# om-ai-lab/OmChat

Hardware: AMD Instinct MI355X
Metric: images/sec prefill + decode tokens/sec, OmChat-13B TP=1/8; p50 TTFT (higher is better)
Workload: dtype bf16

## Files before the change

### include/omchat_hip.h

```cpp
#ifndef OMCHAT_HIP_H
#define OMCHAT_HIP_H
#include <stddef.h>
#include <stdint.h>

#ifdef __cplusplus
extern "C" {
#endif

#define OMCHAT_F16 0
#define OMCHAT_BF16 1
#define OMCHAT_F32 2
#define OMCHAT_PAD_ROW INT32_MIN

typedef struct omchat_ctx omchat_ctx;

typedef struct {
  int v_hidden;
  int v_heads;
  int v_qk_channels;
  int v_mlp;
  int v_layers;
  int v_patch;
  int v_image;
  float v_eps;
// ... 59 lines not shown
int omchat_set_constraints(omchat_ctx* ctx, int b, int no_repeat_ngram_size, int min_new_tokens, int min_length, const int32_t* eos_ids, int n_eos,
                           const int32_t* suppress_ids, int n_suppress, const int32_t* begin_suppress_ids, int n_begin_suppress,
                           const int32_t* bad_word_ids, const int32_t* bad_word_offsets, int n_bad_words, const int32_t* prompt_ids,
                           const int32_t* prompt_len, int max_new, void* stream);
int omchat_set_logprobs(omchat_ctx* ctx, int b, int max_new, void* stream);
int omchat_read_logprobs(omchat_ctx* ctx, int b, float* raw, float* processed, int32_t* counts, int max_len);
#define OMCHAT_LP_MAX_TOP 20
#define OMCHAT_LP_MAX_SCORED 32
int omchat_set_logprobs_ex(omchat_ctx* ctx, int b, int max_new, int top_n, const int32_t* score_ids, int n_score, void* stream);
int omchat_read_logprob_extras(omchat_ctx* ctx, int b, float* top_vals, int32_t* top_ids, float* scored, int32_t* counts, int max_len);
int omchat_read_sampling_state(omchat_ctx* ctx, int row, int* step, uint32_t* seen_words);
int omchat_kv_lengths(omchat_ctx* ctx, int32_t* out, int b);
int omchat_kv_rewind(omchat_ctx* ctx, int b, int n, void* stream);

int omchat_beam_begin(omchat_ctx* ctx, int b, int num_beams, float length_penalty, int early_stopping, const int32_t* eos_ids, int n_eos,
                      int max_new, int prompt_tok_len, void* stream);
int omchat_beam_step(omchat_ctx* ctx, const float* logits, int rows, int32_t* next_tokens, int32_t* done_word, void* stream);
int omchat_beam_result(omchat_ctx* ctx, int num_return, int32_t* tokens, int32_t* lengths, float* scores, int max_len);

int omchat_group_begin(omchat_ctx* ctx, int b, int N, int prompt_len, int share, void* stream);
int omchat_group_share_available(omchat_ctx* ctx, int N);

#define OMCHAT_VERIFY_KEEP_ALL 1
#define OMCHAT_VERIFY_SAMPLE 2
int omchat_decode_verify(omchat_ctx* ctx, const int32_t* tokens, int T, float* logits, int32_t* picks,
                         int* n_accept, int flags, void* stream);

int omchat_prefill_extend(omchat_ctx* ctx, const void* embeds, int S_new, int keep, float* logits_last, void* hidden_out, void* stream);
int omchat_extend_attn_form(int S_new, int keep, int Hkv);
int omchat_kv_read(omchat_ctx* ctx, int layer, int which, int pos0, int n, void* out, void* stream);

int omchat_enable_decode_graph(omchat_ctx* ctx, int on);
int omchat_decode_graph_stats(omchat_ctx* ctx, long* steps, long* replays, long* captures);

int omchat_enable_fp8_decode(omchat_ctx* ctx, int on);

int omchat_enable_mxfp4_decode(omchat_ctx* ctx, int mode);

enum omchat_weight_format {
  OMCHAT_WFMT_16 = 0,
  OMCHAT_WFMT_16_PACKED = 1,
  OMCHAT_WFMT_E4M3 = 2,
  OMCHAT_WFMT_MXFP4 = 3,
  OMCHAT_WFMT_MXFP4_PACKED = 4,
  OMCHAT_WFMT_COUNT = 5
};
int omchat_decode_weight_format(int rows, int fp8_on, int mxfp4_mode, int packed16_ready, int geometry_ok, int* x_pack_nb);

int omchat_enable_fp8_kv(omchat_ctx* ctx, int on);
int omchat_enable_fp8_prefill(omchat_ctx* ctx, int on);

#define OMCHAT_PROF_DECODE_GATEUP 0
#define OMCHAT_PROF_PREFILL_GATEUP 1
#define OMCHAT_PROF_VIT_FC1 2
#define OMCHAT_PROF_CATS 3
int omchat_prof_enable(omchat_ctx* ctx, int on);
int omchat_prof_read(omchat_ctx* ctx, int cat, double* total_ms, long* launches, int reset);

int omchat_mha_fwd(const void* qkv, int B, int S, int H, float softmax_scale, int causal, void* out, int dtype, void* stream);
int omchat_mha_fwd_varlen(const void* qkv, int B, int S, int H, int D, const int32_t* seqlens, float softmax_scale, int causal,
                          void* out, int dtype, void* stream);

int omchat_op_gemm(int dtype, const void* A, int lda, const void* W, int ldw, void* C, int ldc, int M, int N, int K,
                   const void* bias, const void* ls, const void* resid, int ldr, int epi, int force_tile, void* stream);
int omchat_op_gemm_fused(int dtype, const void* A, int lda, const void* W, int ldw, void* C, int ldc, int M, int N, int K,
                         const void* bias, const void* ls, const void* resid, int ldr, int epi, int force_tile, const float* row_scale,
// ... 6 lines not shown
                              int nslots, float* sumsq_q, void* stream);
int omchat_op_mha_qnorm(int dtype, const void* qkv, int B, int Sq, int H, const float* sumsq, int stride, int dim, const void* wq,
                        float eps, float q_scale, void* out, void* stream);
int omchat_op_gemv_norm(int dtype, const void* X, const void* W, int ldw, void* Y, int N, int K, const void* norm_w, float eps,
                        const void* bias, int epi, int out_f32, void* stream);
int omchat_op_set_tuning(int key, int value);
int omchat_gemm_tune_load(const char* path);
int omchat_gemm_tune_dump(const char* path);
long omchat_gemm_tune_runs(void);
size_t omchat_op_gemm_sk_ws(void);
int omchat_op_gemm_sk(int dtype, const void* A, int lda, const void* W, int ldw, void* C, int ldc, int M, int N, int K,
                      const void* bias, const void* ls, const void* resid, int ldr, int epi, int force_tile, void* ws,
                      size_t ws_bytes, int stream_k, void* stream);
int omchat_op_gemv(int dtype, const void* X, int ldx, const void* W, int ldw, void* Y, int ldy, int b, int N, int K,
                   const void* bias, const void* resid, int ldr, int epi, int out_f32, void* stream);
int omchat_op_gemv_packed(int dtype, const void* X, int ldx, const void* W, int ldw, void* Y, int ldy, int b, int N, int K,
                          const void* bias, int epi, int out_f32, int ksplit, int w_packed, int y_packed, void* stream);
int omchat_op_pack_x(int dtype, const void* X, int ldx, int b, int K, void* out, void* stream);
int omchat_op_gemm_fp8(int dtype, const void* A8, const float* a_scale, const void* W8, const float* w_scale, void* C, int ldc, int M, int N,
                       int K, const void* bias, const void* resid, int ldr, int epi, void* stream);
int omchat_op_quant_rows_fp8(int dtype, const void* x, const void* norm_w, float eps, void* y8, float* scale, int rows, int H, void* stream);
int omchat_op_quant_fp8(int dtype, const void* W, int N, int K, void* W8, float* scale, void* stream);
int omchat_op_gemv_fp8(int dtype, const void* X, const void* W8, const float* scale, void* Y, int N, int K, const void* bias,
                       const void* resid, int epi, int out_f32, int ksplit, void* stream);
int omchat_op_quant_mxfp4(int dtype, const void* W, int N, int K, void* W4, void* S, void* stream);
int omchat_op_gemv_mxfp4(int dtype, const void* X, const void* W4, const void* S, void* Y, int N, int K, const void* bias,
                         const void* resid, int epi, int out_f32, int ksplit, void* stream);
int omchat_op_gemv_mxfp4_norm(int dtype, const void* X, const void* W4, const void* S, void* Y, int N, int K, const void* norm_w, float eps,
                              const void* bias, int epi, int out_f32, void* stream);
int omchat_op_gemv_mxfp4_rows(int dtype, const void* X, int ldx, const void* W4, const void* S, void* Y, int ldy, int b, int N, int K,
                              const void* bias, int epi, int out_f32, int ksplit, void* stream);
int omchat_op_gemv_mxfp4_packed(int dtype, const void* X, int ldx, const void* W4, const void* S, void* Y, int ldy, int b, int N, int K,
                                const void* bias, int epi, int out_f32, int ksplit, int y_packed, void* stream);
int omchat_op_pack_w(int dtype, const void* W, int ldw, int N, int K, void* out, void* stream);
int omchat_op_pack_w4(const void* W4, const void* S, int N, int K, void* W4P, void* SP, void* stream);
int omchat_op_gemv_prepacked(int dtype, const void* XP, const void* WP, const void* SP, void* Y, int ldy, int b, int N, int K, const void* bias,
                             int epi, int out_f32, int ksplit, int y_packed, void* stream);
int omchat_op_rmsnorm(int dtype, const void* x, const void* w, void* y, int rows, int H, float eps, void* stream);
int omchat_op_resid_rmsnorm(int dtype, void* x, int ldx, const float* part, int ks, const void* w, void* xn, int ldn, int rows, int H,
                            float eps, int pack_nb, void* stream);
int omchat_op_vit_qknorm(int dtype, void* qkv, int ld, const void* wq, const void* wk, int rows, int C, int C_total,
                         float eps, float q_scale, void* stream);
int omchat_op_attn_prefill(int dtype, const void* q, const void* k, const void* v, void* out, int b, int Sq, int Skv,
                           int Hq, int Hkv, const int32_t* kv_len, int causal, int q_pos0, float scale, void* stream);
int omchat_op_attn_prefill_d(int dtype, const void* q, const void* k, const void* v, void* out, int b, int Sq, int Skv,
                             int Hq, int Hkv, int D, const int32_t* kv_len, int causal, int q_pos0, float scale, void* stream);
int omchat_op_layernorm(int dtype, const void* x, const void* w, const void* b, void* y, int rows, int H, float eps, void* stream);
size_t omchat_op_attn_decode_ws(int b, int Hq, int L);
int omchat_op_attn_decode(int dtype, const void* q, const void* k, const void* v, void* out, int b, int Hq, int Hkv,
                          int cap, int L, const int32_t* kv_len, float scale, void* ws, size_t ws_bytes, void* stream);
int omchat_op_attn_verify(int dtype, const void* q, void* k, void* v, void* out, int T, int Hq, int Hkv, int cap, int L, float scale,
                          void* ws, size_t ws_bytes, void* stream);
int omchat_op_attn_verify_tpw(int keys, int Hkv);
size_t omchat_op_attn_extend_ws(int Sq, int Hq, int Hkv, int L);
int omchat_op_attn_extend(int dtype, const void* q, const void* k, const void* v, void* out, int Sq, int Hq, int Hkv, int cap, int L,
                          float scale, void* ws, size_t ws_bytes, void* stream);
size_t omchat_op_attn_shared_ws(int G, int N, int Hq, int Hkv, int P, int L);
int omchat_op_attn_shared(int dtype, const void* q, void* k, void* v, void* out, int G, int N, int Hq, int Hkv, int cap, int P, int L,
                          float scale, void* ws, size_t ws_bytes, void* stream);
int omchat_op_attn_verify_append(int dtype, const void* qkv, float theta, void* k, void* v, void* out, int T, int Hq, int Hkv, int cap,
                                 int L, float scale, void* ws, size_t ws_bytes, void* stream);
int omchat_op_attn_decode_kv8(int dtype, const void* q, const void* k8, const void* v8, const float* ks, const float* vs, void* out, int b,
                              int Hq, int Hkv, int cap, int L, const int32_t* kv_len, float scale, void* ws, size_t ws_bytes, void* stream);
int omchat_op_attn_decode_kv8_append(int dtype, void* qkv, float theta, void* k8, void* v8, float* ks, float* vs, void* k16, void* v16, void* out,
                                     int b, int Hq, int Hkv, int cap, int L, const int32_t* kv_len, const int32_t* pos, float scale, void* ws,
                                     size_t ws_bytes, void* stream);
// ... 92 lines not shown
```

### omchat_amd/_lib.py

```python
import ctypes as C
import os

HERE = os.path.dirname(os.path.abspath(__file__))
LIB_PATH = os.environ.get("OMCHAT_LIB") or os.path.join(HERE, "lib", "libomchat_hip.so")
_lib = None

F16, BF16, F32 = 0, 1, 2
EPI_NONE, EPI_GELU, EPI_LS_RESID, EPI_RESID, EPI_SWIGLU = 0, 1, 2, 3, 4
EPI_F32OUT = 6
EPI_LS_RESID_STATS, EPI_NONE_STATS = 7, 8
PAD_ROW = -(2 ** 31)
PROF_DECODE_GATEUP, PROF_PREFILL_GATEUP, PROF_VIT_FC1 = 0, 1, 2


class OmchatConfig(C.Structure):
    _fields_ = [
        ("v_hidden", C.c_int), ("v_heads", C.c_int), ("v_qk_channels", C.c_int), ("v_mlp", C.c_int), ("v_layers", C.c_int),
        ("v_patch", C.c_int), ("v_image", C.c_int), ("v_eps", C.c_float),
        ("t_hidden", C.c_int), ("t_layers", C.c_int), ("t_heads", C.c_int), ("t_kv_heads", C.c_int), ("t_mlp", C.c_int),
        ("t_vocab", C.c_int), ("t_vocab_total", C.c_int), ("t_eps", C.c_float), ("rope_theta", C.c_float),
        ("max_seq", C.c_int), ("max_batch", C.c_int), ("max_tiles", C.c_int), ("max_prefill_rows", C.c_int), ("dtype", C.c_int),
        ("v_head_dim", C.c_int), ("v_norm_type", C.c_int), ("v_no_qk_norm", C.c_int),
    ]

# ... 43 lines not shown
    "omchat_decode_step_masked_next": (_i, [_vp, _vp, _i, _vp, _vp, _vp]),
    "omchat_fused_status": (_i, [_vp, C.POINTER(C.c_long), C.POINTER(C.c_uint)]),
    "omchat_has_experiments": (_i, []),
    "omchat_set_allreduce_hook": (_i, [_vp, _vp, _vp]),
    "omchat_allreduce_noop": (_i, [_vp, _vp, C.c_size_t, _i, _vp]),
    "omchat_op_gemv_norm": (_i, [_i, _vp, _vp, _i, _vp, _i, _i, _vp, _f, _vp, _i, _i, _vp]),
    "omchat_prof_enable": (_i, [_vp, _i]),
    "omchat_prof_read": (_i, [_vp, _i, C.POINTER(C.c_double), C.POINTER(C.c_long), _i]),
    "omchat_mha_fwd": (_i, [_vp, _i, _i, _i, _f, _i, _vp, _i, _vp]),
    "omchat_mha_fwd_varlen": (_i, [_vp, _i, _i, _i, _i, _vp, _f, _i, _vp, _i, _vp]),
    "omchat_op_gemm": (_i, [_i, _vp, _i, _vp, _i, _vp, _i, _i, _i, _i, _vp, _vp, _vp, _i, _i, _i, _vp]),
    "omchat_op_gemm_fused": (_i, [_i, _vp, _i, _vp, _i, _vp, _i, _i, _i, _i, _vp, _vp, _vp, _i, _i, _i, _vp, _vp, _i, _i, _i, _f, _vp, _i, _vp, _vp]),
    "omchat_op_stats_finish": (_i, [_vp, _i, _i, _i, _i, _i, _i, _f, _vp, _vp]),
    "omchat_op_row_sumsq": (_i, [_i, _vp, _i, _i, _i, _vp, _vp]),
    "omchat_op_fold_cols": (_i, [_i, _vp, _vp, _vp, _i, _i, _vp]),
    "omchat_op_vit_knorm_slots": (_i, [_i, _vp, _i, _vp, _i, _i, _i, _f, _vp, _i, _i, _vp, _vp]),
    "omchat_op_mha_qnorm": (_i, [_i, _vp, _i, _i, _i, _vp, _i, _i, _vp, _f, _f, _vp, _vp]),
    "omchat_ctx_sp_stats": (_i, [_vp, C.POINTER(C.c_long), C.POINTER(C.c_long)]),
    "omchat_op_set_tuning": (_i, [_i, _i]),
    "omchat_gemm_tune_load": (_i, [C.c_char_p]),
    "omchat_gemm_tune_dump": (_i, [C.c_char_p]),
    "omchat_gemm_tune_runs": (C.c_long, []),
    "omchat_op_gemm_sk_ws": (_sz, []),
    "omchat_op_gemm_sk": (_i, [_i, _vp, _i, _vp, _i, _vp, _i, _i, _i, _i, _vp, _vp, _vp, _i, _i, _i, _vp, _sz, _i, _vp]),
    "omchat_op_gemv": (_i, [_i, _vp, _i, _vp, _i, _vp, _i, _i, _i, _i, _vp, _vp, _i, _i, _i, _vp]),
    "omchat_op_gemv_packed": (_i, [_i, _vp, _i, _vp, _i, _vp, _i, _i, _i, _i, _vp, _i, _i, _i, _i, _i, _vp]),
    "omchat_op_pack_x": (_i, [_i, _vp, _i, _i, _i, _vp, _vp]),
    "omchat_op_gemm_fp8": (_i, [_i, _vp, _vp, _vp, _vp, _vp, _i, _i, _i, _i, _vp, _vp, _i, _i, _vp]),
    "omchat_op_quant_rows_fp8": (_i, [_i, _vp, _vp, _f, _vp, _vp, _i, _i, _vp]),
    "omchat_enable_fp8_decode": (_i, [_vp, _i]),
    "omchat_enable_fp8_kv": (_i, [_vp, _i]),
    "omchat_enable_fp8_prefill": (_i, [_vp, _i]),
    "omchat_enable_decode_graph": (_i, [_vp, _i]),
    "omchat_decode_graph_stats": (_i, [_vp, C.POINTER(C.c_long), C.POINTER(C.c_long), C.POINTER(C.c_long)]),
    "omchat_op_quant_fp8": (_i, [_i, _vp, _i, _i, _vp, _vp, _vp]),
    "omchat_op_gemv_fp8": (_i, [_i, _vp, _vp, _vp, _vp, _i, _i, _vp, _vp, _i, _i, _i, _vp]),
    "omchat_enable_mxfp4_decode": (_i, [_vp, _i]),
    "omchat_decode_weight_format": (_i, [_i, _i, _i, _i, _i, C.POINTER(_i)]),
    "omchat_op_quant_mxfp4": (_i, [_i, _vp, _i, _i, _vp, _vp, _vp]),
    "omchat_op_gemv_mxfp4": (_i, [_i, _vp, _vp, _vp, _vp, _i, _i, _vp, _vp, _i, _i, _i, _vp]),
    "omchat_op_gemv_mxfp4_rows": (_i, [_i, _vp, _i, _vp, _vp, _vp, _i, _i, _i, _i, _vp, _i, _i, _i, _vp]),
    "omchat_op_gemv_mxfp4_packed": (_i, [_i, _vp, _i, _vp, _vp, _vp, _i, _i, _i, _i, _vp, _i, _i, _i, _i, _vp]),
    "omchat_op_pack_w": (_i, [_i, _vp, _i, _i, _i, _vp, _vp]),
    "omchat_op_pack_w4": (_i, [_vp, _vp, _i, _i, _vp, _vp, _vp]),
    "omchat_op_gemv_prepacked": (_i, [_i, _vp, _vp, _vp, _vp, _i, _i, _i, _i, _vp, _i, _i, _i, _i, _vp]),
    "omchat_op_gemv_mxfp4_norm": (_i, [_i, _vp, _vp, _vp, _vp, _i, _i, _vp, _f, _vp, _i, _i, _vp]),
    "omchat_op_rmsnorm": (_i, [_i, _vp, _vp, _vp, _i, _i, _f, _vp]),
    "omchat_op_resid_rmsnorm": (_i, [_i, _vp, _i, _vp, _i, _vp, _vp, _i, _i, _i, _f, _i, _vp]),
    "omchat_op_vit_qknorm": (_i, [_i, _vp, _i, _vp, _vp, _i, _i, _i, _f, _f, _vp]),
    "omchat_op_attn_prefill": (_i, [_i, _vp, _vp, _vp, _vp, _i, _i, _i, _i, _i, _vp, _i, _i, _f, _vp]),
    "omchat_op_attn_prefill_d": (_i, [_i, _vp, _vp, _vp, _vp, _i, _i, _i, _i, _i, _i, _vp, _i, _i, _f, _vp]),
    "omchat_op_layernorm": (_i, [_i, _vp, _vp, _vp, _vp, _i, _i, _f, _vp]),
    "omchat_op_attn_decode_ws": (_sz, [_i, _i, _i]),
    "omchat_op_attn_decode": (_i, [_i, _vp, _vp, _vp, _vp, _i, _i, _i, _i, _i, _vp, _f, _vp, _sz, _vp]),
    "omchat_op_attn_verify_tpw": (_i, [_i, _i]),
    "omchat_op_attn_verify": (_i, [_i, _vp, _vp, _vp, _vp, _i, _i, _i, _i, _i, _f, _vp, _sz, _vp]),
    "omchat_op_attn_extend_ws": (_sz, [_i, _i, _i, _i]),
    "omchat_op_attn_shared_ws": (_sz, [_i, _i, _i, _i, _i, _i]),
    "omchat_op_attn_shared": (_i, [_i, _vp, _vp, _vp, _vp, _i, _i, _i, _i, _i, _i, _i, _f, _vp, _sz, _vp]),
    "omchat_op_attn_extend": (_i, [_i, _vp, _vp, _vp, _vp, _i, _i, _i, _i, _i, _f, _vp, _sz, _vp]),
    "omchat_prefill_extend": (_i, [_vp, _vp, _i, _i, _vp, _vp, _vp]),
    "omchat_extend_attn_form": (_i, [_i, _i, _i]),
    "omchat_kv_read": (_i, [_vp, _i, _i, _i, _i, _vp, _vp]),
    "omchat_op_attn_verify_append": (_i, [_i, _vp, _f, _vp, _vp, _vp, _i, _i, _i, _i, _i, _f, _vp, _sz, _vp]),
    "omchat_op_attn_decode_kv8": (_i, [_i, _vp, _vp, _vp, _vp, _vp, _vp, _i, _i, _i, _i, _i, _vp, _f, _vp, _sz, _vp]),
    "omchat_op_attn_decode_kv8_append": (_i, [_i, _vp, _f, _vp, _vp, _vp, _vp, _vp, _vp, _vp, _i, _i, _i, _i, _i, _vp, _vp, _f, _vp, _sz, _vp]),
    "omchat_op_rope_kv": (_i, [_i, _vp, _i, _i, _i, _i, _i, _f, _vp, _vp, _i, _vp]),
    "omchat_op_rope_kv_q8": (_i, [_i, _vp, _i, _i, _i, _i, _i, _f, _vp, _vp, _i, _vp, _vp, _vp, _vp, _vp]),
    "omchat_op_argmax": (_i, [_vp, _i, _i, _vp, _vp]),
    "omchat_op_attn_prefill_left": (_i, [_i, _vp, _vp, _vp, _vp, _i, _i, _i, _i, _i, _vp, _vp, _i, _i, _f, _i, _vp]),
    "omchat_op_rope_kv_pos": (_i, [_i, _vp, _i, _i, _i, _i, _vp, _i, _i, _i, _f, _vp, _vp, _i, _vp]),
    "omchat_op_argmax_ld": (_i, [_vp, _i, _i, _i, _vp, _vp, _vp, _vp]),
    "omchat_op_im2col": (_i, [_i, _vp, _vp, _i, _i, _i, _i, _vp]),
    "omchat_op_vit_assemble": (_i, [_i, _vp, _vp, _vp, _vp, _i, _i, _i, _vp]),
    "omchat_op_gather_rows": (_i, [_i, _vp, _vp, _vp, _vp, _i, _i, _vp]),
    "omchat_op_copy_rows": (_i, [_i, _vp, _i64, _vp, _i64, _i, _i, _i, _i, _vp]),
    "omchat_op_tp_finish": (_i, [_i, _vp, _vp, _vp, _vp, _vp, _i, _i, _i, _vp]),
    "omchat_op_resid16_norm": (_i, [_i, _vp, _i, _vp, _i, _vp, _vp, _vp, _i, _i, _i, _f, _vp]),
# ... 95 lines not shown
```

### omchat_amd/csrc/capi.hip

```cpp
#include "kernels.h"
#include <stdlib.h>
#include "../../include/omchat_hip.h"
#include <math.h>
#include <vector>

#define S(x) ((hipStream_t)(x))
#if OMCHAT_EXPERIMENTS
int g_launch_any_order = 0;
#endif

extern "C" int omchat_op_gemm(int dtype, const void* A, int lda, const void* W, int ldw, void* C, int ldc, int M, int N, int K,
                              const void* bias, const void* ls, const void* resid, int ldr, int epi, int force_tile, void* stream) {
  GemmArgs g{A, lda, W, ldw, C, ldc, M, N, K, bias, ls, resid, ldr, epi, force_tile, nullptr, 0, -1};
  return launch_gemm(dtype, g, S(stream));
}

extern "C" int omchat_op_gemm_fused(int dtype, const void* A, int lda, const void* W, int ldw, void* C, int ldc, int M, int N, int K,
                                    const void* bias, const void* ls, const void* resid, int ldr, int epi, int force_tile, const float* row_scale,
                                    const float* rs_stats, int rs_ld, int rs_nslots, int rs_dim, float rs_eps,
                                    float* stats, int stats_ld, int* nslots, void* stream) {
  GemmArgs g{A, lda, W, ldw, C, ldc, M, N, K, bias, ls, resid, ldr, epi, force_tile, nullptr, 0, -1};
  g.row_scale = row_scale; g.stats = stats; g.stats_ld = stats_ld; g.stats_nslots = nslots;
  g.rs_stats = rs_stats; g.rs_ld = rs_ld; g.rs_nslots = rs_nslots; g.rs_dim = rs_dim; g.rs_eps = rs_eps;
  return launch_gemm(dtype, g, S(stream));
// ... 39 lines not shown
  if (key == 6) { model_set_pack_replica(value); return 0; }
  if (key == 8) { attn_set_v2(value); return 0; }
  if (key == 9) { model_set_fuse_peer_norm(value); return 0; }
  if (key == 10) { attn_set_tpw(value); return 0; }
  if (key == 11) { gemv_set_no_xs(value); return 0; }
  if (key == 12) { attn_set_klds(value); return 0; }
  if (key == 25) { attn_set_dma(value); return 0; }
  if (key == 26) { attn_set_dma_slots(value); return 0; }
  if (key == 27) { attn_set_dma_rot(value); return 0; }
  if (key == 28) { gemv_set_skew(value); return 0; }
  if (key == 29) { model_set_tp_f32(value); return 0; }
  if (key == 30) { attn_set_hsplit(value); return 0; }
  if (key == 33) { attn_set_mha_xcd(value); return 0; }
  if (key == 16) { gemv_set_norm_loop(value); return 0; }
  if (key == 17) { gemv_set_rows_balance(value); return 0; }
  if (key == 19) { attn_set_merge_mid_min(value); return 0; }
  if (key == 21) { attn_set_merge_dg(value); return 0; }
  if (key == 13) { gemm_set_persist(value); return 0; }
  if (key == 14) { model_set_norm_in_gemv(value); return 0; }
  if (key == 22) { model_set_fuse_attn_oproj(value); return 0; }
  if (key == 23) { model_set_decode_layer(value); return 0; }
  if (key == 24) { gemv_set_dyn(value); return 0; }
  if (key == 34) { gemv_set_shard_shapes(value); return 0; }
  if (key == 35) { model_set_shard_as_tp1(value); return 0; }
  if (key == 36) { attn_set_kg(value); return 0; }
  if (key == 37) { gemm_set_wide_store(value); return 0; }
  if (key == 43) { gemm_set_skip_dead(value); return 0; }
  if (key == 44) { model_set_vit_fused(value); return 0; }
  if (key == 45) { model_set_tp_sp(value); return 0; }
  if (key == 46) { attn_set_peel(value); return 0; }
  if (key == 47) { attn_set_kv8_tpw(value); return 0; }
  if (key == 48) { attn_set_kv8_fuse(value); return 0; }
  if (key == 49) { model_set_extend_attn(value); return 0; }
  if (key == 38) { gemv_set_gu_rr(value); return 0; }
  if (key == 39) { gemv_set_longk_direct(value); return 0; }
  if (key == 40) { norm_set_wave(value); return 0; }
#if OMCHAT_EXPERIMENTS
  if (key == 41) { g_launch_any_order = value; return 0; }
  if (key == 42) { model_set_ao_oproj(value); return 0; }
#endif
  omchat_set_error("omchat_op_set_tuning: unknown key");
  return 1;
}

extern "C" int omchat_allreduce_noop(void*, void*, size_t, int, void*) { return 0; }

extern "C" int omchat_gemm_tune_load(const char* path) { OM_CHECK(path, "null path"); return gemm_tune_load(path); }
extern "C" int omchat_gemm_tune_dump(const char* path) { OM_CHECK(path, "null path"); return gemm_tune_dump(path); }
extern "C" long omchat_gemm_tune_runs(void) { return gemm_tune_runs(); }

extern "C" size_t omchat_op_gemm_sk_ws(void) { return gemm_sk_ws_bytes(); }

extern "C" int omchat_op_gemm_sk(int dtype, const void* A, int lda, const void* W, int ldw, void* C, int ldc, int M, int N, int K,
                                 const void* bias, const void* ls, const void* resid, int ldr, int epi, int force_tile, void* ws,
                                 size_t ws_bytes, int stream_k, void* stream) {
  GemmArgs g{A, lda, W, ldw, C, ldc, M, N, K, bias, ls, resid, ldr, epi, force_tile, ws, ws_bytes, stream_k};
  return launch_gemm(dtype, g, S(stream));
}

extern "C" int omchat_op_gemv(int dtype, const void* X, int ldx, const void* W, int ldw, void* Y, int ldy, int b, int N, int K,
                              const void* bias, const void* resid, int ldr, int epi, int out_f32, void* stream) {
  GemvArgs g{X, ldx, W, ldw, Y, ldy, b, N, K, bias, resid, ldr, epi, out_f32};
  return launch_gemv(dtype, g, S(stream));
}

extern "C" int omchat_op_gemv_norm(int dtype, const void* X, const void* W, int ldw, void* Y, int N, int K, const void* norm_w, float eps,
// ... 635 lines not shown
  if (rc == 0) {
    GemvArgs g{xp, K, wp, K / 2, Y, ldy, b, N, K, bias, nullptr, 0, epi, out_f32, ksplit, 0, nullptr, 1, 1, y_packed};
    g.mx_scale = (const unsigned char*)sp;
    rc = launch_gemv(dtype, g, S(stream));
  }
  hipStreamSynchronize(S(stream));
  drop();
  return rc;
}

extern "C" int omchat_op_pack_w(int dtype, const void* W, int ldw, int N, int K, void* out, void* stream) { return launch_pack_w(dtype, W, ldw, N, K, out, S(stream)); }
extern "C" int omchat_op_pack_w4(const void* W4, const void* S_, int N, int K, void* W4P, void* SP, void* stream) {
  return launch_pack_w4(W4, (const unsigned char*)S_, N, K, W4P, (unsigned char*)SP, S(stream));
}
extern "C" int omchat_op_gemv_prepacked(int dtype, const void* XP, const void* WP, const void* SP, void* Y, int ldy, int b, int N, int K, const void* bias,
                                        int epi, int out_f32, int ksplit, int y_packed, void* stream) {
  OM_CHECK(XP && WP && Y, "null argument");
  OM_CHECK(b >= 1 && b <= 32 && K >= 64 && K % 64 == 0 && N >= 16 && N % 16 == 0, "pre-packed GEMV: 1 <= b <= 32, K % 64 == 0, N % 16 == 0");
  GemvArgs g{XP, K, WP, SP ? K / 2 : K, Y, ldy, b, N, K, bias, nullptr, 0, epi, out_f32, ksplit, 0, nullptr, 1, 1, y_packed};
  g.mx_scale = (const unsigned char*)SP;
  return launch_gemv(dtype, g, S(stream));
}

extern "C" int omchat_op_gemv_mxfp4_norm(int dtype, const void* X, const void* W4, const void* S_, void* Y, int N, int K, const void* norm_w,
                                         float eps, const void* bias, int epi, int out_f32, void* stream) {
  OM_CHECK(X && W4 && S_ && Y && norm_w, "null argument");
  OM_CHECK(K % 32 == 0, "MXFP4: K must be a multiple of 32 (one e8m0 scale per 32 consecutive k)");
  GemvArgs g{X, K, W4, K / 2, Y, N, 1, N, K, bias, nullptr, 0, epi, out_f32};
  g.norm_w = norm_w; g.norm_eps = eps;
  g.mx_scale = (const unsigned char*)S_;
  return launch_gemv(dtype, g, S(stream));
}

extern "C" int omchat_op_attn_prefill_d(int dtype, const void* q, const void* k, const void* v, void* out, int b, int Sq, int Skv, int Hq,
                                        int Hkv, int D, const int32_t* kv_len, int causal, int q_pos0, float scale, void* stream) {
  AttnArgs a{};
  a.Q = q; a.q_sb = (int64_t)Sq * Hq * D; a.q_sh = D; a.q_sr = (int64_t)Hq * D;
  a.K = k; a.k_sb = (int64_t)Hkv * Skv * D; a.k_sh = (int64_t)Skv * D; a.k_sr = D;
  a.V = v; a.v_sb = a.k_sb; a.v_sh = a.k_sh; a.v_sr = D;
  a.O = out; a.o_sb = a.q_sb; a.o_sh = D; a.o_sr = a.q_sr;
  a.batch = b; a.q_heads = Hq; a.kv_heads = Hkv; a.Sq = Sq; a.Skv = Skv; a.kv_len = kv_len; a.causal = causal; a.q_pos0 = q_pos0; a.scale = scale;
  a.head_dim = D;
  return launch_attn_prefill(dtype, a, S(stream));
}

extern "C" int omchat_op_layernorm(int dtype, const void* x, const void* w, const void* b, void* y, int rows, int H, float eps, void* stream) {
  return launch_layernorm(dtype, x, H, w, b, y, H, rows, H, eps, S(stream));
}

extern "C" int omchat_op_attn_prefill_left(int dtype, const void* q, const void* k, const void* v, void* out, int b, int Sq, int Skv, int Hq,
                                           int Hkv, const int32_t* kv_len, const int32_t* kv_start, int causal, int q_pos0, float scale,
                                           int fill_uniform, void* stream) {
  OM_CHECK(q && k && v && out && kv_start, "null argument");
  AttnArgs a{};
  a.Q = q; a.q_sb = (int64_t)Sq * Hq * 128; a.q_sh = 128; a.q_sr = (int64_t)Hq * 128;
  a.K = k; a.k_sb = (int64_t)Hkv * Skv * 128; a.k_sh = (int64_t)Skv * 128; a.k_sr = 128;
  a.V = v; a.v_sb = a.k_sb; a.v_sh = a.k_sh; a.v_sr = 128;
  a.O = out; a.o_sb = a.q_sb; a.o_sh = 128; a.o_sr = a.q_sr;
  a.batch = b; a.q_heads = Hq; a.kv_heads = Hkv; a.Sq = Sq; a.Skv = Skv; a.kv_len = kv_len; a.kv_start = kv_start; a.causal = causal;
  a.q_pos0 = q_pos0; a.scale = scale;
  int rc = launch_attn_prefill(dtype, a, S(stream));
  if (!rc && fill_uniform) rc = launch_attn_uniform_rows(dtype, a, S(stream));
  return rc;
}

extern "C" int omchat_op_rope_kv_pos(int dtype, void* qkv, int b, int Sq, int Hq, int Hkv, const int32_t* pos, int pos0, int slot0, int max_pos,
// ... 76 lines not shown
```

### omchat_amd/csrc/ctx.h

```cpp
#pragma once
#include "kernels.h"
#include "../../include/omchat_hip.h"
#include <rccl/rccl.h>
#include <string>
#include <unordered_map>
#include <vector>

#define TRY(x) do { int rc_ = (x); if (rc_) return rc_; } while (0)

extern int g_fuse_peer_norm;

enum RouteKind { R_PLAIN = 0, R_GATE = 1, R_UP = 2, R_PATCH = 3 };
struct Route {
  void* dst = nullptr;
  int64_t rows = 0, cols = 0;
  int64_t dst_ld = 0;
  int kind = R_PLAIN;
  bool loaded = false;
  float synth_std = 0.02f, synth_off = 0.f;
};

struct Grown {
  void* p = nullptr; size_t cap = 0;
  void release() { if (p) (void)hipFree(p); p = nullptr; cap = 0; }
// ... 64 lines not shown
};

struct GroupState {
  bool share = false; int b = 0, N = 0, P = 0;
  Grown ws;
  std::vector<int> hpos, hlen;
  bool on() const { return share; }
  void end() { share = false; }
  void release() { ws.release(); }
};

struct omchat_ctx {
  omchat_config c;
  int dt = OMCHAT_BF16;
  int tp_rank = 0, tp_size = 1;
  ncclComm_t comm = nullptr;
  std::vector<void*> allocs;
  size_t bytes = 0;
  std::unordered_map<std::string, Route> routes;

  int v_np = 0, v_ntok = 0, v_Cq = 0, v_kpad = 0, v_hd = 128;
  int t_qdim = 0, t_kvdim = 0, t_qkvdim = 0;

  struct VitLayer { void *ls1, *ls2, *n1, *n2, *n1b, *n2b, *wqkv, *qn, *kn, *wproj, *bproj, *w1, *b1, *w2, *b2; };
  struct DecLayer { void *ln1, *ln2, *wqkv, *bqkv, *wo, *wgu, *wd; };
  enum Proj { P_QKV = 0, P_O = 1, P_GU = 2, P_DOWN = 3, P_LM = 4 };
  struct WRef { void* W = nullptr; int ldw = 0; float* w_scale = nullptr; unsigned char* mx_scale = nullptr; int packed = 0; };
  enum WState { W_ABSENT = 0, W_BUILT, W_STALE, W_UNAVAILABLE };
  struct WTable { std::vector<WRef> e; int state = W_ABSENT; };
  WTable wt[OMCHAT_WFMT_COUNT];
  const WRef* layer_w(int fmt, int layer) const { return &wt[fmt].e[(size_t)layer * 4]; }
  const WRef& lm_w(int fmt) const { return wt[fmt].e.back(); }
  bool built(int fmt) const { return wt[fmt].state == W_BUILT; }
  bool fp8_decode = false;
  int mxfp4_mode = 0;
  void *k8cache = nullptr, *v8cache = nullptr;
  float *ks8 = nullptr, *vs8 = nullptr;
  bool fp8_kv = false, kv8_valid = false, fp8_prefill = false;
  void* tw_q8 = nullptr; float* tw_q8s = nullptr;
  int64_t scale_layer_stride() const { return (int64_t)c.max_batch * c.t_kv_heads * c.max_seq; }
  struct DecodeGraph { hipGraph_t graph = nullptr; hipGraphExec_t exec = nullptr; int cap_len = 0, grp_N = 0, grp_P = 0; const void* grp_ws = nullptr; };
  std::unordered_map<int, DecodeGraph> graphs;
  bool graph_on = false;
  hipStream_t graph_stream = nullptr;
  hipEvent_t graph_ev_in = nullptr, graph_ev_out = nullptr;
  int32_t *d_tok_in = nullptr, *d_tok_out = nullptr;
  long graph_steps = 0, graph_replays = 0, graph_captures = 0;
  void *v_cls = nullptr, *v_pos = nullptr, *v_wpatch = nullptr, *v_bpatch = nullptr;
  std::vector<VitLayer> vl;
  void *p_w0 = nullptr, *p_b0 = nullptr, *p_w2 = nullptr, *p_b2 = nullptr;
  void *t_embed = nullptr, *t_norm = nullptr, *t_lm = nullptr;
  std::vector<DecLayer> dl;
  float* rope = nullptr;

  void *vw_cols = nullptr, *vw_pe = nullptr, *vw_x = nullptr, *vw_x2 = nullptr, *vw_xn = nullptr, *vw_qkv = nullptr, *vw_ao = nullptr,
       *vw_h = nullptr, *vw_feat = nullptr, *vw_proj = nullptr;
  float* vw_sumsq = nullptr;
  float *vw_stats_x = nullptr, *vw_stats_qk = nullptr, *vw_rstd = nullptr;
  int vw_stats_x_ld = 0, vw_stats_qk_ld = 0, vw_stats_x_ld_used = 1;
  struct VitFold { void *wqkv = nullptr, *w1 = nullptr; };
  std::vector<VitFold> vfold;
  bool vfold_stale = true;
  void *tw_x = nullptr, *tw_x2 = nullptr, *tw_xn = nullptr, *tw_qkv = nullptr, *tw_ao = nullptr, *tw_act = nullptr, *tw_last = nullptr;
  float* tw_logits = nullptr;
  void* sk_ws = nullptr; size_t sk_ws_bytes = 0;
  float* tp_f32_ws = nullptr; size_t tp_f32_bytes = 0;
// ... 123 lines not shown
    if (sp_peer(blk * tp_size * 2)) { ++n_ar_peer; return omchat_peer_reduce_scatter(peer, buf, blk, dt, s); }
    if (!sp_native(blk * tp_size * 2)) return allreduce_any(buf, blk * tp_size, dt, s);
    ++n_ar_rccl;
    ncclResult_t r = ncclReduceScatter(buf, (char*)buf + (size_t)tp_rank * blk * 2, blk, dt == OMCHAT_F16 ? ncclFloat16 : ncclBfloat16, ncclSum, comm, s);
    if (r != ncclSuccess) { omchat_set_error(std::string("ncclReduceScatter: ") + ncclGetErrorString(r)); return 3; }
    return 0;
  }
  int all_gather_rows(void* buf, int blk_rows, int N, hipStream_t s) {
    if (tp_size == 1) return 0;
    ++n_ag;
    const size_t blk = (size_t)blk_rows * N;
    if (sp_peer(blk * tp_size * 2)) { ++n_ar_peer; return omchat_peer_all_gather(peer, buf, blk, dt, s); }
    if (!sp_native(blk * tp_size * 2)) {
      if (hook == omchat_allreduce_noop) return 0;
      if (tp_rank > 0 && hipMemsetAsync(buf, 0, (size_t)tp_rank * blk * 2, s) != hipSuccess) { omchat_set_error("all_gather_rows: memset"); return 2; }
      if (tp_rank + 1 < tp_size && hipMemsetAsync((char*)buf + (size_t)(tp_rank + 1) * blk * 2, 0, (size_t)(tp_size - 1 - tp_rank) * blk * 2, s) != hipSuccess) {
        omchat_set_error("all_gather_rows: memset"); return 2;
      }
      return allreduce_any(buf, blk * tp_size, dt, s);
    }
    ++n_ar_rccl;
    ncclResult_t r = ncclAllGather((char*)buf + (size_t)tp_rank * blk * 2, buf, blk, dt == OMCHAT_F16 ? ncclFloat16 : ncclBfloat16, comm, s);
    if (r != ncclSuccess) { omchat_set_error(std::string("ncclAllGather: ") + ncclGetErrorString(r)); return 3; }
    return 0;
  }
  int allreduce(void* buf, size_t count, hipStream_t s) { return allreduce_any(buf, count, dt, s); }
  int allreduce_f32(float* buf, size_t count, hipStream_t s) { return allreduce_any(buf, count, OMCHAT_F32, s); }
};

inline void use_weight(GemvArgs& g, const omchat_ctx::WRef& w) {
  g.W = w.W; g.ldw = w.ldw; g.w_scale = w.w_scale; g.mx_scale = w.mx_scale; g.w_packed = w.packed;
}

void drop_decode_graphs(omchat_ctx* ctx);

int pick_alloc(omchat_ctx* ctx, int rows);
int pick_admit(omchat_ctx* ctx, bool picks, bool feeds);
int greedy_pick(omchat_ctx* ctx, const float* lg, int b, int32_t* next_tokens, hipStream_t s, bool advance = false);
int pick_run(omchat_ctx* ctx, const float* lg, int b, int32_t* next_tokens, hipStream_t s, bool advance = false, const int32_t* fed = nullptr,
             bool force_greedy = false);
int pick_verify(omchat_ctx* ctx, const float* lg, int T, const int32_t* tokens, int32_t* picks, hipStream_t s, bool sample);
const char* pick_verify_refusal(omchat_ctx* ctx, int flags);
int pick_verify_prepare(omchat_ctx* ctx);
void pick_verify_committed(omchat_ctx* ctx, int n_picks);
int pick_feed(omchat_ctx* ctx, const int32_t* fed, int b, hipStream_t s);
const char* pick_rewind_refusal(omchat_ctx* ctx, int b, int n);
int pick_rewind(omchat_ctx* ctx, int b, int n, hipStream_t s);
```

### omchat_amd/csrc/gemv.hip

```cpp
#include "kernels.h"
#include "rowdot.h"
#include <type_traits>

namespace {

struct GemvP {
  const void* X; const void* W; void* Y; const void* bias; const void* resid;
  int ldx, ldw, ldy, ldr, b, N, K, out_f32, ksplit;
  const float* w_scale;
  int y_packed;
  const void* norm_w; float norm_eps;
  unsigned* dyn;
  void* y_pack;
  unsigned long long* dbg;
  const unsigned char* mx_s;
#if OMCHAT_EXPERIMENTS
  int xskew;
#endif
};
constexpr int WF_16 = 0, WF_E4M3 = 1, WF_MX4 = 2;
#if OMCHAT_EXPERIMENTS
#define OM_DBG_MIN(slot, cond) do { if (p.dbg && (cond) && threadIdx.x == 0) atomicMax(p.dbg + (slot), ~wall_clock64()); } while (0)
#define OM_DBG_MAX(slot, cond) do { if (p.dbg && (cond) && threadIdx.x == 0) atomicMax(p.dbg + (slot), wall_clock64()); } while (0)
#else
#define OM_DBG_MIN(slot, cond) do { } while (0)
#define OM_DBG_MAX(slot, cond) do { } while (0)
#endif

template <typename T, int NTILE, int N, int WAVES, bool NTL, int NB>
__device__ __forceinline__ void gemv_group(f32x4 (&acc)[NTILE][NB], const T* const (&wrow)[NTILE], const T* const (&xrow)[NB], int k0,
                                           const bool (&xvalid)[NB]) {
  typedef typename V8<T>::type frag_t;
  frag_t wf[N][NTILE][2], xf[N][NB][2];
#pragma unroll
  for (int u = 0; u < N; ++u) {
    const int k = k0 + u * WAVES * 64;
#pragma unroll
    for (int t = 0; t < NTILE; ++t) {
      if constexpr (NTL) {
        wf[u][t][0] = __builtin_nontemporal_load(reinterpret_cast<const frag_t*>(wrow[t] + k));
        wf[u][t][1] = __builtin_nontemporal_load(reinterpret_cast<const frag_t*>(wrow[t] + k + 32));
      } else {
        wf[u][t][0] = ld8<T>(wrow[t] + k);
        wf[u][t][1] = ld8<T>(wrow[t] + k + 32);
      }
    }
#pragma unroll
    for (int nb = 0; nb < NB; ++nb) {
      xf[u][nb][0] = ld8<T>(xrow[nb] + k);
      xf[u][nb][1] = ld8<T>(xrow[nb] + k + 32);
    }
  }
  frag_t zero;
// ... 569 lines not shown
  const unsigned w0 = w.x, w1 = w.y, x0 = x.x, x1 = x.y, x2 = x.z, x3 = x.w;
  acc = __builtin_amdgcn_fdot2(__builtin_amdgcn_cvt_scalef32_pk_f16_fp8(w0, 1.0f, false), __builtin_bit_cast(v2, x0), acc, false);
  acc = __builtin_amdgcn_fdot2(__builtin_amdgcn_cvt_scalef32_pk_f16_fp8(w0, 1.0f, true), __builtin_bit_cast(v2, x1), acc, false);
  acc = __builtin_amdgcn_fdot2(__builtin_amdgcn_cvt_scalef32_pk_f16_fp8(w1, 1.0f, false), __builtin_bit_cast(v2, x2), acc, false);
  acc = __builtin_amdgcn_fdot2(__builtin_amdgcn_cvt_scalef32_pk_f16_fp8(w1, 1.0f, true), __builtin_bit_cast(v2, x3), acc, false);
  return acc;
}

template <typename T> __device__ __forceinline__ float rw_dot8_fp4(unsigned w, rw_u32x4 x);
template <> __device__ __forceinline__ float rw_dot8_fp4<bf16>(unsigned w, rw_u32x4 x) {
  typedef bf16 v2 __attribute__((ext_vector_type(2)));
  const unsigned x0 = x.x, x1 = x.y, x2 = x.z, x3 = x.w;
  float acc = 0.f;
  acc = __builtin_amdgcn_fdot2_f32_bf16(__builtin_amdgcn_cvt_scalef32_pk_bf16_fp4(w, 1.0f, 0), __builtin_bit_cast(v2, x0), acc, false);
  acc = __builtin_amdgcn_fdot2_f32_bf16(__builtin_amdgcn_cvt_scalef32_pk_bf16_fp4(w, 1.0f, 1), __builtin_bit_cast(v2, x1), acc, false);
  acc = __builtin_amdgcn_fdot2_f32_bf16(__builtin_amdgcn_cvt_scalef32_pk_bf16_fp4(w, 1.0f, 2), __builtin_bit_cast(v2, x2), acc, false);
  acc = __builtin_amdgcn_fdot2_f32_bf16(__builtin_amdgcn_cvt_scalef32_pk_bf16_fp4(w, 1.0f, 3), __builtin_bit_cast(v2, x3), acc, false);
  return acc;
}
template <> __device__ __forceinline__ float rw_dot8_fp4<f16>(unsigned w, rw_u32x4 x) {
  typedef f16 v2 __attribute__((ext_vector_type(2)));
  const unsigned x0 = x.x, x1 = x.y, x2 = x.z, x3 = x.w;
  float acc = 0.f;
  acc = __builtin_amdgcn_fdot2(__builtin_amdgcn_cvt_scalef32_pk_f16_fp4(w, 1.0f, 0), __builtin_bit_cast(v2, x0), acc, false);
  acc = __builtin_amdgcn_fdot2(__builtin_amdgcn_cvt_scalef32_pk_f16_fp4(w, 1.0f, 1), __builtin_bit_cast(v2, x1), acc, false);
  acc = __builtin_amdgcn_fdot2(__builtin_amdgcn_cvt_scalef32_pk_f16_fp4(w, 1.0f, 2), __builtin_bit_cast(v2, x2), acc, false);
  acc = __builtin_amdgcn_fdot2(__builtin_amdgcn_cvt_scalef32_pk_f16_fp4(w, 1.0f, 3), __builtin_bit_cast(v2, x3), acc, false);
  return acc;
}

template <int WF> struct RwW { typedef rw_u32x4 type; };
template <> struct RwW<WF_E4M3> { typedef rw_u32x2 type; };
template <> struct RwW<WF_MX4> { typedef rw_u32x2 type; };
template <typename T, int WF>
__device__ __forceinline__ typename RwW<WF>::type rw_ldw(const GemvP& p, size_t row, int k) {
  if constexpr (WF == WF_E4M3) {
    return __builtin_nontemporal_load(reinterpret_cast<const rw_u32x2*>((const unsigned char*)p.W + row * p.ldw + k));
  } else if constexpr (WF == WF_MX4) {
    rw_u32x2 w;
    w.x = __builtin_nontemporal_load(reinterpret_cast<const unsigned*>((const unsigned char*)p.W + row * p.ldw + (k >> 1)));
    w.y = __builtin_nontemporal_load(p.mx_s + row * (size_t)(p.K >> 5) + (k >> 5));
    return w;
  } else {
    return __builtin_nontemporal_load(reinterpret_cast<const rw_u32x4*>((const T*)p.W + row * p.ldw + k));
  }
}
template <typename T, int WF>
__device__ __forceinline__ float rw_dotw(typename RwW<WF>::type w, rw_u32x4 x, float acc) {
  if constexpr (WF == WF_E4M3) return rw_dot8_fp8<T>(w, x, acc);
  else if constexpr (WF == WF_MX4) return fmaf(rw_dot8_fp4<T>(w.x, x), mx_scale_of(w.y), acc);
  else return rw_dot8<T>(w, x, acc);
}

template <typename T, int R> struct RwTail { const T* p0; const T* p1; int idx[R]; float v0[R], v1[R]; };
template <typename T, int R> __device__ __forceinline__ void rw_tail_load(RwTail<T, R>& t) {
#pragma unroll
  for (int r = 0; r < R; ++r) { t.v0[r] = tof(t.p0[t.idx[r]]); t.v1[r] = tof(t.p1[t.idx[r]]); }
}
template <typename T, int R, int NCH, int WF>
__device__ __forceinline__ void rw_rows_q(const GemvP& p, const int (&rows)[R], int k0, int lane, const rw_u32x4 (&xr)[RW_MAXC], float (&acc)[R],
                                          RwTail<T, R>& tail) {
  typename RwW<WF>::type w[R][NCH];
#pragma unroll
  for (int r = 0; r < R; ++r)
#pragma unroll
    for (int c = 0; c < NCH; ++c) {
      int k = k0 + c * 512 + lane * 8;
      k = k < p.K ? k : k0;
// ... 167 lines not shown
    const bool ok = c < NCH && k < p.K;
    xq[i] = ok ? *reinterpret_cast<const rw_u32x4*>((const T*)p.X + k) : z;
    nq[i] = ok ? *reinterpret_cast<const rw_u32x4*>((const T*)p.norm_w + k) : z;
  }
#pragma unroll
  for (int i = 0; i < SC; ++i) {
    if constexpr (WAVES == 4) {
      sq[i] = xq[i];
    } else {
      const int c = wave + 4 * i, k = c * 512 + lane * 8;
      const rw_u32x4 z = {0u, 0u, 0u, 0u};
      sq[i] = (wave < 4 && c < NCH && k < p.K) ? *reinterpret_cast<const rw_u32x4*>((const T*)p.X + k) : z;
    }
  }
  int rows[R];
#pragma unroll
  for (int r = 0; r < R; ++r) {
    if constexpr (EPI == EPI_SWIGLU) {
      int n = g * RR + (r % RR); n = n < n_out ? n : n_out - 1;
      rows[r] = 32 * (n >> 4) + (n & 15) + (r / RR) * 16;
    } else {
      const int n = g * R + r;
      rows[r] = n < p.N ? n : p.N - 1;
    }
  }
  typedef typename RwW<F8>::type wreg_t;
  wreg_t w[R][NCH];
#pragma unroll
  for (int r = 0; r < R; ++r)
#pragma unroll
    for (int c = 0; c < NCH; ++c) {
      int k = c * 512 + lane * 8;
      k = k < p.K ? k : 0;
      w[r][c] = rw_ldw<T, F8>(p, (size_t)rows[r], k);
    }
  float e_bias[RR], e_scale[R];
  {
    const T* bp = (EPI != EPI_SWIGLU && p.bias) ? (const T*)p.bias : (const T*)p.norm_w;
    const int nmax = (EPI != EPI_SWIGLU && p.bias) ? n_out - 1 : 0;
#pragma unroll
    for (int r = 0; r < RR; ++r) {
      const int n = g * RR + r;
      e_bias[r] = tof(bp[n < nmax ? n : nmax]);
    }
    if (!(EPI != EPI_SWIGLU && p.bias)) {
#pragma unroll
      for (int r = 0; r < RR; ++r) e_bias[r] = 0.f;
    }
#pragma unroll
    for (int r = 0; r < R; ++r) e_scale[r] = 1.f;
    if constexpr (F8 == WF_E4M3) {
#pragma unroll
      for (int r = 0; r < R; ++r) e_scale[r] = p.w_scale[rows[r]];
    }
  }
  __builtin_amdgcn_sched_barrier(0);
  float ss = 0.f;
#pragma unroll
  for (int i = 0; i < SC; ++i) {
    const v8 xv = __builtin_bit_cast(v8, sq[i]);
#pragma unroll
    for (int j = 0; j < 8; ++j) { const float v = tof(xv[j]); ss += v * v; }
  }
#pragma unroll
  for (int o = 32; o > 0; o >>= 1) ss += __shfl_xor(ss, o, 64);
  if (lane == 0 && wave < 4) red[wave] = ss;
  asm volatile("s_waitcnt lgkmcnt(0)" ::: "memory");
  __builtin_amdgcn_s_barrier();
  float tot = red[0];
#pragma unroll
  for (int w = 1; w < 4; ++w) tot += red[w];
  const float inv = rsqrtf(tot / (float)p.K + p.norm_eps);
#pragma unroll
  for (int i = 0; i < MC; ++i) {
    const int c = wave + WAVES * i;
    if (c < NCH) {
      const v8 xv = __builtin_bit_cast(v8, xq[i]), wv = __builtin_bit_cast(v8, nq[i]);
      v8 o;
#pragma unroll
      for (int j = 0; j < 8; ++j) o[j] = fromf<T>(tof(wv[j]) * rnd<T>(tof(xv[j]) * inv));
      *reinterpret_cast<v8*>(xs + c * 512 + lane * 8) = o;
    }
  }
  asm volatile("s_waitcnt lgkmcnt(0)" ::: "memory");
  __builtin_amdgcn_s_barrier();
  rw_u32x4 xr[NCH];
#pragma unroll
  for (int c = 0; c < NCH; ++c) xr[c] = *reinterpret_cast<const rw_u32x4*>(xs + c * 512 + lane * 8);
  __builtin_amdgcn_sched_barrier(0);
  float acc[R];
#pragma unroll
  for (int r = 0; r < R; ++r) {
    float a = 0.f;
#pragma unroll
    for (int c = 0; c < NCH; ++c) {
      a = rw_dotw<T, F8>(w[r][c], xr[c], a);
    }
#pragma unroll
    for (int o = 32; o > 0; o >>= 1) a += __shfl_xor(a, o, 64);
    if constexpr (F8 == WF_E4M3) a *= e_scale[r];
    acc[r] = a;
  }
  if (lane == 0) {
#pragma unroll
    for (int r = 0; r < RR; ++r) {
      const int n = g * RR + r;
      if (n >= n_out) continue;
      if constexpr (EPI == EPI_SWIGLU) {
        const float gt = rnd<T>(acc[r]), up = rnd<T>(acc[r + RR]);
        ((T*)p.Y)[n] = fromf<T>(rnd<T>(silu(gt)) * up);
      } else {
        const float y = acc[r] + e_bias[r];
        if (p.out_f32) ((float*)p.Y)[n] = y;
        else ((T*)p.Y)[n] = fromf<T>(y);
      }
    }
  }
  if constexpr (EPI == EPI_SWIGLU) { OM_DBG_MAX(5, blockIdx.x + 64 >= gridDim.x); OM_DBG_MAX(16 + (blockIdx.x & 7), blockIdx.x + 512 >= gridDim.x); }
  if constexpr (EPI == EPI_NONE) OM_DBG_MAX(9, (blockIdx.x & 7) == 0);
}

template <typename T, int EPI, int RR, int NCH, bool F8, int WAVES = 4>
__global__ __launch_bounds__(WAVES * 64) void gemv_rows_norm_kernel(GemvP p) { gemv_rows_norm_body<T, EPI, RR, NCH, F8 ? WF_E4M3 : WF_16, WAVES>(p); }
template <typename T, int EPI, int RR, int NCH, int WAVES = 4>
__global__ __launch_bounds__(WAVES * 64) void gemv_rows_norm_mx4_kernel(GemvP p) { gemv_rows_norm_body<T, EPI, RR, NCH, WF_MX4, WAVES>(p); }

template <typename T, int EPI, int NCH, int F8>
__device__ __forceinline__ void gemv_rows_norm_loop_body(const GemvP& p, int per_wg, unsigned skew) {
  typedef typename V8<T>::type v8;
  constexpr int R = EPI == EPI_SWIGLU ? 2 : 1;
  __shared__ __attribute__((aligned(16))) T xs[NCH * 512];
  __shared__ float red[4];
  const int lane = threadIdx.x & 63, wave = __builtin_amdgcn_readfirstlane(threadIdx.x >> 6);
  const int n_out = EPI == EPI_SWIGLU ? p.N / 2 : p.N;
  int o0 = blockIdx.x * per_wg, o1 = o0 + per_wg < n_out ? o0 + per_wg : n_out;
  if constexpr (EPI == EPI_SWIGLU) OM_DBG_MIN(4, blockIdx.x < 8);
  if (skew) {
    const int l = blockIdx.x & 7;
    int pre = 0;
    for (int i = 0; i < l; ++i) pre += per_wg + (int)((skew >> (4 * i)) & 15u) - 8;
    o0 = (blockIdx.x >> 3) * 8 * per_wg + pre;
    o1 = o0 + per_wg + (int)((skew >> (4 * l)) & 15u) - 8;
    o1 = o1 < n_out ? o1 : n_out;
  }
  typedef typename RwW<F8>::type wreg_t;
  auto row_of = [&](int n, int r) { return EPI == EPI_SWIGLU ? 32 * (n >> 4) + (n & 15) + r * 16 : n; };
  auto load_w = [&](wreg_t (&w)[R][NCH], int n) {
#pragma unroll
    for (int r = 0; r < R; ++r) {
      const size_t row = (size_t)row_of(n, r);
#pragma unroll
      for (int c = 0; c < NCH; ++c) {
        int k = c * 512 + lane * 8;
        k = k < p.K ? k : 0;
        w[r][c] = rw_ldw<T, F8>(p, row, k);
      }
    }
  };
// ... 233 lines not shown
    if (out_ok(nx3, 1)) load_w(wb, nx3 * DYN_CH + 1);
    if (out_ok(cur, 1)) finish(wc, cur * DYN_CH + 1);
    cur = nx3;
  }
  if (lane == 0) {
    const unsigned done = __hip_atomic_fetch_add(p.dyn + 64 * DYN_POOLS, 1u, __ATOMIC_RELAXED, __HIP_MEMORY_SCOPE_AGENT);
    if (done == gridDim.x * 4u - 1u) {
      for (int i = 0; i <= DYN_POOLS; ++i) __hip_atomic_store(p.dyn + 64 * i, 0u, __ATOMIC_RELAXED, __HIP_MEMORY_SCOPE_AGENT);
    }
  }
}

template <typename T, int EPI, int NCH, bool F8>
__global__ __launch_bounds__(256) void gemv_rows_norm_dyn_kernel(GemvP p) { gemv_rows_norm_dyn_body<T, EPI, NCH, F8 ? WF_E4M3 : WF_16>(p); }
template <typename T, int EPI, int NCH>
__global__ __launch_bounds__(256) void gemv_rows_norm_dyn_mx4_kernel(GemvP p) { gemv_rows_norm_dyn_body<T, EPI, NCH, WF_MX4>(p); }

template <typename T, int F8>
__device__ __forceinline__ void gemv_rows_longk_body(const GemvP& p, int rows_per_wg) {
  extern __shared__ __attribute__((aligned(16))) char xs_raw[];
  T* xs = (T*)xs_raw;
  const int lane = threadIdx.x & 63, wave = __builtin_amdgcn_readfirstlane(threadIdx.x >> 6);
  const int nch = (p.K + 511) >> 9, npass = (nch + 7) >> 3;
  const int n = blockIdx.x * rows_per_wg + wave;
  const bool valid = n < p.N;
  const int row = valid ? n : p.N - 1;
  OM_DBG_MIN(6, blockIdx.x < 8);
  typedef typename RwW<F8>::type wreg_t;
  auto load_w = [&](wreg_t (&w)[8], int pass) {
#pragma unroll
    for (int c = 0; c < 8; ++c) {
      int k = (pass * 8 + c) * 512 + lane * 8;
      k = k < p.K ? k : 0;
      w[c] = rw_ldw<T, F8>(p, (size_t)row, k);
    }
  };
  float acc = 0.f;
  auto dots = [&](wreg_t (&w)[8], int pass) {
#pragma unroll
    for (int c = 0; c < 8; ++c) {
      const rw_u32x4 xr = *reinterpret_cast<const rw_u32x4*>(xs + (pass * 8 + c) * 512 + lane * 8);
      acc = rw_dotw<T, F8>(w[c], xr, acc);
    }
  };
  wreg_t wa[8], wb[8], wc[8];
  load_w(wa, 0);
  if (npass > 1) load_w(wb, 1);
  if (npass > 2) load_w(wc, 2);
  const float e_bias_raw = tof(((const T*)(p.bias ? p.bias : p.X))[p.bias ? row : 0]);
  const float e_res_raw = tof(((const T*)(p.resid ? p.resid : p.X))[p.resid ? row : 0]);
  const float e_bias = p.bias ? e_bias_raw : 0.f, e_res = p.resid ? e_res_raw : 0.f;
  float e_scale = 1.f;
  if constexpr (F8 == WF_E4M3) e_scale = p.w_scale[row];
  for (int i = threadIdx.x; i < npass * 8 * 64; i += blockDim.x) {
    const rw_u32x4 z = {0u, 0u, 0u, 0u};
    const rw_u32x4 v = i * 8 < p.K ? *reinterpret_cast<const rw_u32x4*>((const T*)p.X + i * 8) : z;
    *reinterpret_cast<rw_u32x4*>(xs + i * 8) = v;
  }
  __syncthreads();
  for (int ps = 0; ps < npass; ps += 3) {
    if (ps > 0 && ps + 2 < npass) load_w(wc, ps + 2);
    dots(wa, ps);
    if (ps + 1 < npass) {
      if (ps + 3 < npass) load_w(wa, ps + 3);
      dots(wb, ps + 1);
    }
    if (ps + 2 < npass) {
      if (ps + 4 < npass) load_w(wb, ps + 4);
      dots(wc, ps + 2);
    }
  }
  float a = acc;
#pragma unroll
  for (int o = 32; o > 0; o >>= 1) a += __shfl_xor(a, o, 64);
  if constexpr (F8 == WF_E4M3) a *= e_scale;
  if (lane == 0 && valid) {
    const float y = rnd<T>(a + e_bias);
    ((T*)p.Y)[n] = fromf<T>(e_res + y);
  }
  OM_DBG_MAX(7, (blockIdx.x & 7) == 0);
}

template <typename T, bool F8>
__global__ __launch_bounds__(512) void gemv_rows_longk_kernel(GemvP p, int rows_per_wg) { gemv_rows_longk_body<T, F8 ? WF_E4M3 : WF_16>(p, rows_per_wg); }
template <typename T>
__global__ __launch_bounds__(512) void gemv_rows_longk_mx4_kernel(GemvP p, int rows_per_wg) { gemv_rows_longk_body<T, WF_MX4>(p, rows_per_wg); }

#if OMCHAT_EXPERIMENTS
template <typename T, int F8>
__device__ __forceinline__ void gemv_rows_longk_direct_body(const GemvP& p) {
  const int lane = threadIdx.x & 63, wave = __builtin_amdgcn_readfirstlane(threadIdx.x >> 6);
  const int nch = (p.K + 511) >> 9, npass = (nch + 7) >> 3;
  const int n = blockIdx.x * (int)(blockDim.x >> 6) + wave;
  if (n >= p.N) return;
  const int row = n;
  typedef typename RwW<F8>::type wreg_t;
  auto load_w = [&](wreg_t (&w)[8], int pass) {
#pragma unroll
    for (int c = 0; c < 8; ++c) {
      int k = (pass * 8 + c) * 512 + lane * 8;
      k = k < p.K ? k : 0;
      w[c] = rw_ldw<T, F8>(p, (size_t)row, k);
    }
  };
  auto load_x = [&](rw_u32x4 (&x)[8], int pass) {
#pragma unroll
    for (int c = 0; c < 8; ++c) {
      const int k = (pass * 8 + c) * 512 + lane * 8;
      const rw_u32x4 z = {0u, 0u, 0u, 0u};
      x[c] = k < p.K ? *reinterpret_cast<const rw_u32x4*>((const T*)p.X + k) : z;
    }
  };
  float acc = 0.f;
  auto dots = [&](wreg_t (&w)[8], rw_u32x4 (&x)[8]) {
#pragma unroll
    for (int c = 0; c < 8; ++c) {
      acc = rw_dotw<T, F8>(w[c], x[c], acc);
    }
  };
// ... 20 lines not shown
  for (int o = 32; o > 0; o >>= 1) a += __shfl_xor(a, o, 64);
  if constexpr (F8 == WF_E4M3) a *= e_scale;
  if (lane == 0) {
    const float y = rnd<T>(a + e_bias);
    ((T*)p.Y)[n] = fromf<T>(e_res + y);
  }
}

template <typename T, bool F8>
__global__ __launch_bounds__(256) void gemv_rows_longk_direct_kernel(GemvP p) { gemv_rows_longk_direct_body<T, F8 ? WF_E4M3 : WF_16>(p); }
template <typename T>
__global__ __launch_bounds__(256) void gemv_rows_longk_direct_mx4_kernel(GemvP p) { gemv_rows_longk_direct_body<T, WF_MX4>(p); }

#endif
int g_gemv_longk_direct = 0;

template <typename T>
int launch_rows_longk(const GemvP& p, hipStream_t s) {
#if OMCHAT_EXPERIMENTS
  if (g_gemv_longk_direct > 0) {
    const int wpw = g_gemv_longk_direct > 4 ? 4 : g_gemv_longk_direct;
    if (p.mx_s) hipLaunchKernelGGL((gemv_rows_longk_direct_mx4_kernel<T>), dim3(cdiv(p.N, wpw)), dim3(64 * wpw), 0, s, p);
    else if (p.w_scale) hipLaunchKernelGGL((gemv_rows_longk_direct_kernel<T, true>), dim3(cdiv(p.N, wpw)), dim3(64 * wpw), 0, s, p);
    else hipLaunchKernelGGL((gemv_rows_longk_direct_kernel<T, false>), dim3(cdiv(p.N, wpw)), dim3(64 * wpw), 0, s, p);
    return 0;
  }
#endif
  const int n_cu = device_cus();
  int rpw = cdiv(p.N, 2 * n_cu);
  rpw = rpw < 1 ? 1 : (rpw > 8 ? 8 : rpw);
  const int grid = cdiv(p.N, rpw);
  const int npass = (cdiv(p.K, 512) + 7) / 8;
  const size_t lds = (size_t)npass * 8 * 512 * 2;
  if (p.mx_s) {
    static PerDeviceOnce set;
    auto k = gemv_rows_longk_mx4_kernel<T>;
    if (set.first()) OM_HIP(hipFuncSetAttribute((const void*)k, hipFuncAttributeMaxDynamicSharedMemorySize, 64 * 1024));
    hipLaunchKernelGGL(k, dim3(grid), dim3(64 * rpw), lds, s, p, rpw);
  } else if (p.w_scale) {
    auto k = gemv_rows_longk_kernel<T, true>;
    static PerDeviceOnce set;
    if (set.first()) OM_HIP(hipFuncSetAttribute((const void*)k, hipFuncAttributeMaxDynamicSharedMemorySize, 64 * 1024));
    hipLaunchKernelGGL(k, dim3(grid), dim3(64 * rpw), lds, s, p, rpw);
  } else {
    auto k = gemv_rows_longk_kernel<T, false>;
    static PerDeviceOnce set;
    if (set.first()) OM_HIP(hipFuncSetAttribute((const void*)k, hipFuncAttributeMaxDynamicSharedMemorySize, 64 * 1024));
    hipLaunchKernelGGL(k, dim3(grid), dim3(64 * rpw), lds, s, p, rpw);
  }
  return 0;
}

int g_gemv_rows_balance = 1;
unsigned g_gemv_skew = 0;
int g_gemv_dyn = 0;
int g_gemv_gu_rr = 1;
int g_gemv_gu_rr8 = 1;
int g_gemv_norm_loop = 0;

template <typename T, int EPI, int RR, int F8, int NCH>
void launch_rows_norm_n(const GemvP& p, hipStream_t s) {
  const int n_out = EPI == EPI_SWIGLU ? p.N / 2 : p.N;
  if constexpr (NCH >= 4) {
    const bool want = EPI == EPI_SWIGLU ? (g_gemv_norm_loop & (F8 != WF_16 ? 4 : 1)) : (p.N < 32768 ? (g_gemv_norm_loop & 2) : (g_gemv_norm_loop & 8));
    const int n_cu = device_cus();
#if OMCHAT_EXPERIMENTS
    if (want && p.dyn && g_gemv_dyn && n_out >= 8 * n_cu) {
// ... 16 lines not shown
      if constexpr (F8 == WF_MX4) hipLaunchKernelGGL((gemv_rows_norm_mx4_kernel<T, EPI, 1, NCH, 9>), dim3(2 * n_cu), dim3(576), 0, s, p);
      else hipLaunchKernelGGL((gemv_rows_norm_kernel<T, EPI, 1, NCH, F8 == WF_E4M3, 9>), dim3(2 * n_cu), dim3(576), 0, s, p);
      return;
    }
  }
#if OMCHAT_EXPERIMENTS
  if constexpr (EPI == EPI_SWIGLU && RR == 1) {
    const int nwg = cdiv(n_out, 4), xs = (int)(g_gemv_skew < 256u ? g_gemv_skew : 0u);
    if (xs > 0 && nwg % 8 == 0 && n_out % 4 == 0 && xs < nwg / 8) {
      GemvP q = p; q.xskew = xs;
      if constexpr (F8 == WF_MX4) hipLaunchKernelGGL((gemv_rows_norm_mx4_kernel<T, EPI, RR, NCH>), dim3(8 * (nwg / 8 + xs)), dim3(256), 0, s, q);
      else hipLaunchKernelGGL((gemv_rows_norm_kernel<T, EPI, RR, NCH, F8 == WF_E4M3>), dim3(8 * (nwg / 8 + xs)), dim3(256), 0, s, q);
      return;
    }
  }
#endif
  if constexpr (F8 == WF_MX4) hipLaunchKernelGGL((gemv_rows_norm_mx4_kernel<T, EPI, RR, NCH>), dim3(cdiv(cdiv(n_out, RR), 4)), dim3(256), 0, s, p);
  else hipLaunchKernelGGL((gemv_rows_norm_kernel<T, EPI, RR, NCH, F8 == WF_E4M3>), dim3(cdiv(cdiv(n_out, RR), 4)), dim3(256), 0, s, p);
}
template <typename T, int EPI, int RR, int F8>
void launch_rows_norm(const GemvP& p, hipStream_t s) {
  switch (cdiv(p.K, 512)) {
    case 1: launch_rows_norm_n<T, EPI, RR, F8, 1>(p, s); break;
    case 2: launch_rows_norm_n<T, EPI, RR, F8, 2>(p, s); break;
    case 3: launch_rows_norm_n<T, EPI, RR, F8, 3>(p, s); break;
    case 4: launch_rows_norm_n<T, EPI, RR, F8, 4>(p, s); break;
    case 5: launch_rows_norm_n<T, EPI, RR, F8, 5>(p, s); break;
    case 6: launch_rows_norm_n<T, EPI, RR, F8, 6>(p, s); break;
    case 7: launch_rows_norm_n<T, EPI, RR, F8, 7>(p, s); break;
    default: launch_rows_norm_n<T, EPI, RR, F8, 8>(p, s); break;
  }
}

template <typename T, int EPI, int RR, int F8>
void launch_rows_r(const GemvP& p, hipStream_t s) {
  const int n_out = EPI == EPI_SWIGLU ? p.N / 2 : p.N;
  if constexpr (RR == 1 && EPI == EPI_RESID) {
    const int n_cu = device_cus();
    if (g_gemv_rows_balance && p.ksplit == 1 && n_out == 7 * 2 * n_cu) {
      if constexpr (F8 == WF_MX4) hipLaunchKernelGGL((gemv_rows_mx4_kernel<T, EPI, 1, 7>), dim3(2 * n_cu, 1), dim3(448), 0, s, p);
      else hipLaunchKernelGGL((gemv_rows_kernel<T, EPI, 1, 7, F8 == WF_E4M3>), dim3(2 * n_cu, 1), dim3(448), 0, s, p);
      return;
    }
  }
  int grid = cdiv(cdiv(n_out, RR), 4);
  grid = grid > 2048 ? 2048 : grid;
  if constexpr (F8 == WF_MX4) hipLaunchKernelGGL((gemv_rows_mx4_kernel<T, EPI, RR, 4>), dim3(grid, p.ksplit), dim3(256), 0, s, p);
  else hipLaunchKernelGGL((gemv_rows_kernel<T, EPI, RR, 4, F8 == WF_E4M3>), dim3(grid, p.ksplit), dim3(256), 0, s, p);
}
template <typename T, int EPI, int WF>
void launch_rows_q(const GemvP& p, hipStream_t s) {
  if constexpr (EPI == EPI_SWIGLU || EPI == EPI_NONE) {
    if (p.norm_w) {
      if (EPI == EPI_NONE && p.N < 32768) launch_rows_norm<T, EPI, 2, WF>(p, s);
      else if (EPI == EPI_SWIGLU && g_gemv_gu_rr8 == 2) launch_rows_norm<T, EPI, 2, WF>(p, s);
      else if (EPI == EPI_SWIGLU && g_gemv_gu_rr8 == 1) launch_rows_norm<T, EPI, 1, WF>(p, s);
      else launch_rows_norm<T, EPI, 4, WF>(p, s);
      return;
    }
  }
  if ((EPI == EPI_NONE || EPI == EPI_RESID) && p.N < 32768) launch_rows_r<T, EPI, 1, WF>(p, s);
  else if (EPI == EPI_NONE) launch_rows_r<T, EPI, 8, WF>(p, s);
  else launch_rows_r<T, EPI, 4, WF>(p, s);
}
template <typename T, int EPI>
void launch_rows(const GemvP& p, hipStream_t s) {
  if (p.mx_s) { launch_rows_q<T, EPI, WF_MX4>(p, s); return; }
  if (p.w_scale) { launch_rows_q<T, EPI, WF_E4M3>(p, s); return; }
  if constexpr (EPI == EPI_SWIGLU || EPI == EPI_NONE) {
    if (p.norm_w) {
      if (EPI == EPI_NONE && p.N < 32768) launch_rows_norm<T, EPI, 2, WF_16>(p, s);
      else if (EPI == EPI_SWIGLU && g_gemv_gu_rr == 2) launch_rows_norm<T, EPI, 2, WF_16>(p, s);
      else if (EPI == EPI_SWIGLU && g_gemv_gu_rr == 3) launch_rows_norm<T, EPI, 3, WF_16>(p, s);
      else if (EPI == EPI_SWIGLU) launch_rows_norm<T, EPI, 1, WF_16>(p, s);
      else launch_rows_norm<T, EPI, 4, WF_16>(p, s);
      return;
    }
  }
  if ((EPI == EPI_NONE || EPI == EPI_RESID) && p.N < 32768) launch_rows_r<T, EPI, 1, WF_16>(p, s);
  else if (EPI == EPI_SWIGLU && (g_gemv_shard & 4) && p.N / 2 < 16 * device_cus()) launch_rows_r<T, EPI, 1, WF_16>(p, s);
  else launch_rows_r<T, EPI, 4, WF_16>(p, s);
}

template <typename T>
int launch_t(const GemvArgs& a, hipStream_t s) {
  const int ks = a.ksplit > 1 ? a.ksplit : 1;
  GemvP p{a.X, a.W, a.Y, a.bias, a.resid, a.ldx, a.ldw, a.ldy, a.ldr, a.b, a.N, a.K, a.out_f32, ks, a.w_scale, a.y_packed, a.norm_w, a.norm_eps,
          (unsigned*)a.dyn_ctr, a.y_pack, a.dbg, a.mx_scale};
  if (a.norm_w && a.x_packed && !(a.w_packed && ks == 1 && (a.K >> 6) == 56 && a.epi == EPI_SWIGLU && a.N % 32 == 0 && !g_gemv_no_xs)) {
    omchat_set_error("launch_gemv: the in-register RMSNorm on packed x exists for the x-stationary gate|up form only (packed W, K = 3584, no split-K)");
    return 1;
  }
  if (a.epi == EPI_RESID && a.x_packed && !(a.w_packed && ks == 1 && (a.K >> 6) == 56 && a.N % 16 == 0 && a.N / 16 <= device_cus() && !g_gemv_no_xs)) {
    omchat_set_error("launch_gemv: the batched residual epilogue exists for the x-stationary form only (packed W, K = 3584, N / 16 <= CUs, no split-K)");
    return 1;
  }
  if (a.x_packed) {
#define OM_PK(NT_, EPI_, WV_, UN_)                                                                                                  \
  do {                                                                                                                              \
    const dim3 grid(cdiv(cdiv(a.N, 16), NT_), ks);                                                                                  \
    if (a.mx_scale) { if (a.b > 16) hipLaunchKernelGGL((gemv_pk_mx4_kernel<T, NT_, EPI_, WV_, UN_, 2>), grid, dim3(WV_ * 64), 0, s, p);     \
                      else hipLaunchKernelGGL((gemv_pk_mx4_kernel<T, NT_, EPI_, WV_, UN_, 1>), grid, dim3(WV_ * 64), 0, s, p); }             \
    else if (a.b > 16) { if (a.w_packed) hipLaunchKernelGGL((gemv_pk_kernel<T, NT_, EPI_, WV_, UN_, 2, true>), grid, dim3(WV_ * 64), 0, s, p);   \
                    else hipLaunchKernelGGL((gemv_pk_kernel<T, NT_, EPI_, WV_, UN_, 2, false>), grid, dim3(WV_ * 64), 0, s, p); }            \
    else { if (a.w_packed) hipLaunchKernelGGL((gemv_pk_kernel<T, NT_, EPI_, WV_, UN_, 1, true>), grid, dim3(WV_ * 64), 0, s, p);            \
           else hipLaunchKernelGGL((gemv_pk_kernel<T, NT_, EPI_, WV_, UN_, 1, false>), grid, dim3(WV_ * 64), 0, s, p); }                     \
  } while (0)
    const int n_cu = device_cus();
    if (a.mx_scale && (a.norm_w || a.epi == EPI_RESID)) {
      omchat_set_error("launch_gemv: the batched norm-in-GEMV / residual forms read 16-bit weights only (no MXFP4 instantiation)");
      return 1;
    }
#if !OMCHAT_EXPERIMENTS
    if (a.norm_w || a.epi == EPI_RESID) { omchat_set_error("launch_gemv: the batched norm-in-GEMV / residual forms need a -DOMCHAT_EXPERIMENTS=1 build"); return 1; }
#else
    if (a.w_packed && ks == 1 && !g_gemv_no_xs && (a.K >> 6) == 56 && a.epi == EPI_RESID) {
      const dim3 grid(a.N / 16);
      if (a.b > 16) hipLaunchKernelGGL((gemv_xs_kernel<T, EPI_RESID, 2, 7>), grid, dim3(512), 0, s, p);
      else hipLaunchKernelGGL((gemv_xs_kernel<T, EPI_RESID, 1, 7>), grid, dim3(512), 0, s, p);
      OM_LAUNCH_CHECK();
      return 0;
// ... 31 lines not shown
      const int q = (a.K >> 6) / 8;
      int a5 = -1;
      for (int t = 0; t <= ks; ++t) if (5 * t + 2 * (ks - t) == q) a5 = t;
      const int n_cu2 = device_cus();
      int gx = std::max(1, n_cu2 / ks);
      const int tiles = a.N / 16;
      if (tiles < 4 * gx && tiles % 2 == 0 && (long)tiles * ks >= n_cu2 && (long)tiles * ks <= 2L * n_cu2) gx = tiles / 2;
      if (a5 >= 0 && (tiles >= 4 * gx || gx == tiles / 2)) {
        const dim3 grid(gx, ks);
        if (a.mx_scale) {
          if (a.b > 16) hipLaunchKernelGGL((gemv_xs_split_mx4_kernel<T, 2>), grid, dim3(512), 0, s, p, a5);
          else hipLaunchKernelGGL((gemv_xs_split_mx4_kernel<T, 1>), grid, dim3(512), 0, s, p, a5);
        } else if (a.b > 16) hipLaunchKernelGGL((gemv_xs_split_kernel<T, 2>), grid, dim3(512), 0, s, p, a5);
        else hipLaunchKernelGGL((gemv_xs_split_kernel<T, 1>), grid, dim3(512), 0, s, p, a5);
        OM_LAUNCH_CHECK();
        return 0;
      }
    }
    if (a.norm_w) { omchat_set_error("launch_gemv: packed-x RMSNorm form: gate|up shape outside the x-stationary launch (N / 32 >= 4 CUs)"); return 1; }
    if (a.epi == EPI_SWIGLU) OM_PK(2, EPI_SWIGLU, 8, 4);
    else if (a.epi == EPI_PARTIAL) {
      const int cps = cdiv(a.K >> 6, ks);
      if ((g_gemv_shard & 2) && cps <= 8) OM_PK(1, EPI_PARTIAL, 8, 1);
      else if ((g_gemv_shard & 2) && cps <= 32) OM_PK(1, EPI_PARTIAL, 8, 2);
      else if (a.K / ks >= 1536) OM_PK(4, EPI_PARTIAL, 4, 2);
      else OM_PK(2, EPI_PARTIAL, 8, 4);
    }
    else if (a.N >= 32768) OM_PK(4, EPI_NONE, 4, 4);
    else OM_PK(2, EPI_NONE, 8, 4);
#undef OM_PK
    OM_LAUNCH_CHECK();
    return 0;
  }
  if (a.b == 1 && !a.x_packed && a.epi == EPI_RESID && ks == 1 && !a.out_f32 && a.K > RW_MAXC * 512 && a.K % 8 == 0 && a.K <= 32768 &&
      ((!a.force_mfma && !g_gemv_force_mfma) || a.mx_scale)) {
    const int rc = launch_rows_longk<T>(p, s);
    if (rc) return rc;
    OM_LAUNCH_CHECK();
    return 0;
  }
  const bool rows_ok = a.b == 1 && cdiv(cdiv(a.K, 512), ks) <= RW_MAXC;
  if (a.norm_w && !(rows_ok && ks == 1 && !a.force_mfma && !g_gemv_force_mfma && (a.epi == EPI_NONE || a.epi == EPI_SWIGLU))) {
    omchat_set_error("launch_gemv: the in-register RMSNorm needs the whole-row batch-1 form without split-K (K <= 4096), epilogue NONE / SWIGLU");
    return 1;
  }
  if ((a.w_scale || a.mx_scale) && !rows_ok) { omchat_set_error("launch_gemv: fp8 / MXFP4 weights need b == 1 and <= 8 chunks of 512 per K slice"); return 1; }
  if (rows_ok && (a.w_scale || a.mx_scale || (!a.force_mfma && !g_gemv_force_mfma))) {
    switch (a.epi) {
      case EPI_PARTIAL: launch_rows<T, EPI_PARTIAL>(p, s); break;
      case EPI_SWIGLU: launch_rows<T, EPI_SWIGLU>(p, s); break;
      case EPI_RESID: launch_rows<T, EPI_RESID>(p, s); break;
      default: launch_rows<T, EPI_NONE>(p, s); break;
    }
    OM_LAUNCH_CHECK();
    return 0;
  }
  if (a.b > 16) {
    if (a.epi == EPI_PARTIAL) hipLaunchKernelGGL((gemv_kernel<T, 1, EPI_PARTIAL, 8, 4, false, 2>), dim3(cdiv(a.N, 16), ks), dim3(512), 0, s, p);
    else if (a.epi == EPI_SWIGLU) hipLaunchKernelGGL((gemv_kernel<T, 2, EPI_SWIGLU, 8, 4, false, 2>), dim3(cdiv(a.N, 32)), dim3(512), 0, s, p);
    else if (a.epi == EPI_RESID) hipLaunchKernelGGL((gemv_kernel<T, 1, EPI_RESID, 8, 4, false, 2>), dim3(cdiv(a.N, 16)), dim3(512), 0, s, p);
    else hipLaunchKernelGGL((gemv_kernel<T, 2, EPI_NONE, 8, 4, false, 2>), dim3(cdiv(a.N, 32)), dim3(512), 0, s, p);
    OM_LAUNCH_CHECK();
    return 0;
  }
  if (a.epi == EPI_PARTIAL) {
    if (a.K / 64 / ks <= 32)
      hipLaunchKernelGGL((gemv_kernel<T, 1, EPI_PARTIAL, 4, 8>), dim3(cdiv(a.N, 16), ks), dim3(256), 0, s, p);
    else
      hipLaunchKernelGGL((gemv_kernel<T, 1, EPI_PARTIAL, 8, 4>), dim3(cdiv(a.N, 16), ks), dim3(512), 0, s, p);
  } else if (a.epi == EPI_SWIGLU) {
    hipLaunchKernelGGL((gemv_kernel<T, 2, EPI_SWIGLU, 8, 4>), dim3(cdiv(a.N, 32)), dim3(512), 0, s, p);
  } else if (a.epi == EPI_RESID) {
    hipLaunchKernelGGL((gemv_kernel<T, 1, EPI_RESID, 8, 4>), dim3(cdiv(a.N, 16)), dim3(512), 0, s, p);
  } else {
    if (a.N >= 16384)
      hipLaunchKernelGGL((gemv_kernel<T, 2, EPI_NONE, 8, 8>), dim3(cdiv(a.N, 32)), dim3(512), 0, s, p);
    else
      hipLaunchKernelGGL((gemv_kernel<T, 1, EPI_NONE, 8, 8>), dim3(cdiv(a.N, 16)), dim3(512), 0, s, p);
  }
  OM_LAUNCH_CHECK();
  return 0;
}

}

void gemv_set_force_mfma(int v) { g_gemv_force_mfma = v; }
int gemv_get_force_mfma() { return g_gemv_force_mfma; }
void gemv_set_no_xs(int v) { g_gemv_no_xs = v; }
void gemv_set_shard_shapes(int v) { g_gemv_shard = v; }
int gemv_get_shard_shapes() { return g_gemv_shard; }
void gemv_set_norm_loop(int v) { g_gemv_norm_loop = v; }
void gemv_set_gu_rr(int v) { if (v >= 16) g_gemv_gu_rr8 = v / 16; else g_gemv_gu_rr = v; }
void gemv_set_dyn(int v) { g_gemv_dyn = v; }
void gemv_set_longk_direct(int v) { g_gemv_longk_direct = v; }
void gemv_set_skew(int v) { g_gemv_skew = (unsigned)v; }
void gemv_set_rows_balance(int v) { g_gemv_rows_balance = v; }

namespace {
template <typename T>
__global__ __launch_bounds__(256) void quant_fp8_rows_kernel(const T* __restrict__ W, int ldw, int N, int K, unsigned char* __restrict__ W8, int ldq,
                                                             float* __restrict__ scale) {
  const int lane = threadIdx.x & 63, n = blockIdx.x * 4 + (threadIdx.x >> 6);
  if (n >= N) return;
  const T* w = W + (size_t)n * ldw;
  float m = 0.f;
  for (int k = lane * 8; k < K; k += 512) {
    const typename V8<T>::type v = ld8<T>(w + k);
#pragma unroll
    for (int j = 0; j < 8; ++j) m = fmaxf(m, fabsf(tof(v[j])));
  }
#pragma unroll
  for (int o = 32; o > 0; o >>= 1) m = fmaxf(m, __shfl_xor(m, o, 64));
  const float sc = m > 0.f ? m / 448.0f : 1.0f;
  if (lane == 0) scale[n] = sc;
  for (int k = lane * 8; k < K; k += 512) {
    const typename V8<T>::type v = ld8<T>(w + k);
    float f[8];
#pragma unroll
    for (int j = 0; j < 8; ++j) f[j] = tof(v[j]) / sc;
    int lo = 0, hi = 0;
    lo = __builtin_amdgcn_cvt_pk_fp8_f32(f[0], f[1], lo, false);
    lo = __builtin_amdgcn_cvt_pk_fp8_f32(f[2], f[3], lo, true);
    hi = __builtin_amdgcn_cvt_pk_fp8_f32(f[4], f[5], hi, false);
    hi = __builtin_amdgcn_cvt_pk_fp8_f32(f[6], f[7], hi, true);
    rw_u32x2 o2 = {(unsigned)lo, (unsigned)hi};
    *reinterpret_cast<rw_u32x2*>(W8 + (size_t)n * ldq + k) = o2;
  }
}
}
// ... 18 lines not shown
    const typename V8<T>::type v = ld8<T>(w + k);
    float f[8], m = 0.f;
#pragma unroll
    for (int j = 0; j < 8; ++j) { f[j] = tof(v[j]); m = fmaxf(m, fabsf(f[j])); }
    m = fmaxf(m, __shfl_xor(m, 1, 64));
    m = fmaxf(m, __shfl_xor(m, 2, 64));
    const int field = (int)((__float_as_uint(m) >> 23) & 0xffu);
    int e = field - 127 - 2;
    e = e < -127 ? -127 : e;
    if (m == 0.f) e = 0;
    const float inv = ldexpf(1.0f, -e);
    unsigned codes = 0;
#pragma unroll
    for (int j = 0; j < 8; ++j) {
      const float a = fabsf(f[j]) * inv;
      const unsigned c = (unsigned)(a > 0.25f) + (unsigned)(a >= 0.75f) + (unsigned)(a > 1.25f) + (unsigned)(a >= 1.75f) + (unsigned)(a > 2.5f) +
                         (unsigned)(a >= 3.5f) + (unsigned)(a > 5.0f);
      const unsigned sgn = (c != 0u && f[j] < 0.f) ? 8u : 0u;
      codes |= (c | sgn) << (4 * j);
    }
    *reinterpret_cast<unsigned*>(W4 + (size_t)n * ld4 + (k >> 1)) = codes;
    if ((lane & 3) == 0) S[(size_t)n * (K >> 5) + (k >> 5)] = (unsigned char)(e + 127);
  }
}
}

int launch_quant_mxfp4_rows(int dtype, const void* W, int ldw, int N, int K, void* W4, int ld4, unsigned char* S, hipStream_t s) {
  OM_CHECK(W && W4 && S, "null argument");
  OM_CHECK(N >= 1 && K >= 32 && K % 32 == 0, "MXFP4: K must be a multiple of 32 (one e8m0 scale per 32 consecutive k)");
  OM_CHECK(ldw % 8 == 0 && ld4 % 4 == 0 && ld4 >= K / 2, "ldw % 8, ld4 (bytes) % 4 and >= K / 2");
  if (dtype == OMCHAT_F16) hipLaunchKernelGGL(quant_mxfp4_rows_kernel<f16>, dim3(cdiv(N, 4)), dim3(256), 0, s, (const f16*)W, ldw, N, K, (unsigned char*)W4, ld4, S);
  else if (dtype == OMCHAT_BF16) hipLaunchKernelGGL(quant_mxfp4_rows_kernel<bf16>, dim3(cdiv(N, 4)), dim3(256), 0, s, (const bf16*)W, ldw, N, K, (unsigned char*)W4, ld4, S);
  else { omchat_set_error("launch_quant_mxfp4_rows: bad dtype"); return 1; }
  OM_LAUNCH_CHECK();
  return 0;
}

int launch_pack_x(int dtype, const void* X, int ldx, int b, int K, void* out, hipStream_t s) {
  OM_CHECK(b >= 1 && b <= 32 && K % 64 == 0 && ldx % 8 == 0, "pack_x: 1 <= b <= 32, K % 64, ldx % 8");
  const int NB = b > 16 ? 2 : 1;
  const int grid = cdiv(NB * 16 * (K / 8), 256);
  if (dtype == OMCHAT_F16) hipLaunchKernelGGL(pack_x_kernel<f16>, dim3(grid), dim3(256), 0, s, (const f16*)X, ldx, b, K, (f16*)out, NB);
  else if (dtype == OMCHAT_BF16) hipLaunchKernelGGL(pack_x_kernel<bf16>, dim3(grid), dim3(256), 0, s, (const bf16*)X, ldx, b, K, (bf16*)out, NB);
  else { omchat_set_error("launch_pack_x: bad dtype"); return 1; }
  OM_LAUNCH_CHECK();
  return 0;
}

int launch_pack_w4(const void* W4, const unsigned char* S, int N, int K, void* W4P, unsigned char* SP, hipStream_t s) {
  OM_CHECK(W4 && S && W4P && SP, "null argument");
  OM_CHECK(N >= 16 && N % 16 == 0, "pack_w4: N % 16 == 0 (16-row weight tiles)");
  OM_CHECK(K >= 64 && K % 64 == 0, "pack_w4: K % 64 == 0 (64-wide K chunks)");
  const long n8 = (long)N * (K / 8);
  const int grid = (int)(cdiv64(n8, 256) > 8192 ? 8192 : cdiv64(n8, 256));
  hipLaunchKernelGGL(pack_w4_kernel, dim3(grid), dim3(256), 0, s, (const unsigned char*)W4, S, N, K, (unsigned*)W4P, SP);
  OM_LAUNCH_CHECK();
  return 0;
}

int launch_pack_w(int dtype, const void* W, int ldw, int N, int K, void* out, hipStream_t s) {
  OM_CHECK(N % 16 == 0 && K % 64 == 0 && ldw % 8 == 0, "pack_w: N % 16, K % 64, ldw % 8");
  const long n8 = (long)N * (K / 8);
  const int grid = (int)(cdiv64(n8, 256) > 8192 ? 8192 : cdiv64(n8, 256));
  if (dtype == OMCHAT_F16) hipLaunchKernelGGL(pack_w_kernel<f16>, dim3(grid), dim3(256), 0, s, (const f16*)W, ldw, N, K, (f16*)out);
  else if (dtype == OMCHAT_BF16) hipLaunchKernelGGL(pack_w_kernel<bf16>, dim3(grid), dim3(256), 0, s, (const bf16*)W, ldw, N, K, (bf16*)out);
  else { omchat_set_error("launch_pack_w: bad dtype"); return 1; }
// ... 96 lines not shown
```

### omchat_amd/csrc/kernels.h

```cpp
#pragma once
#ifndef OMCHAT_EXPERIMENTS
#define OMCHAT_EXPERIMENTS 0
#endif
#include "common.h"
#if OMCHAT_EXPERIMENTS
#include <hip/hip_ext.h>
extern int g_launch_any_order;
#undef hipLaunchKernelGGL
#define hipLaunchKernelGGL(kernelName, numBlocks, numThreads, memPerBlock, streamId, ...)                                                      \
  do {                                                                                                                                         \
    if (g_launch_any_order)                                                                                                                    \
      hipExtLaunchKernelGGL((kernelName), dim3(numBlocks), dim3(numThreads), (memPerBlock), (streamId), nullptr, nullptr, hipExtAnyOrderLaunch, \
                            __VA_ARGS__);                                                                                                      \
    else                                                                                                                                       \
      hipLaunchKernelGGLInternal((kernelName), numBlocks, numThreads, memPerBlock, streamId, __VA_ARGS__);                                     \
  } while (0)
#endif

enum {
  EPI_NONE = 0,
  EPI_GELU = 1,
  EPI_LS_RESID = 2,
  EPI_RESID = 3,
  EPI_SWIGLU = 4,
// ... 20 lines not shown
  const float* row_scale = nullptr;
  const float* rs_stats = nullptr; int rs_ld = 0, rs_nslots = 0, rs_dim = 0; float rs_eps = 0.f;
  float* stats = nullptr; int stats_ld = 0; int* stats_nslots = nullptr;
};
int launch_gemm(int dtype, const GemmArgs& a, hipStream_t stream);
int launch_stats_finish(const float* stats, int ld, int slot0, int nslots, int ngroups, int rows, int dim, float eps, float* out, hipStream_t s);
int launch_row_sumsq(int dtype, const void* x, int ldx, int rows, int H, float* stats, hipStream_t s);
size_t gemm_sk_ws_bytes();
void gemm_set_skew(int v);
void gemm_set_persist(int v);
void gemm_set_wide_store(int v);
void gemm_set_skip_dead(int v);

struct GemvArgs {
  const void* X; int ldx;
  const void* W; int ldw;
  void* Y; int ldy;
  int b, N, K;
  const void* bias;
  const void* resid; int ldr;
  int epi;
  int out_f32;
  int ksplit;
  int force_mfma;
  const float* w_scale;
  int x_packed;
  int w_packed;
  int y_packed;
  const void* norm_w; float norm_eps;
  void* dyn_ctr = nullptr;
  void* y_pack = nullptr;
  unsigned long long* dbg = nullptr;
  const unsigned char* mx_scale = nullptr;
};
int launch_pack_x(int dtype, const void* X, int ldx, int b, int K, void* out, hipStream_t s);
int launch_pack_w(int dtype, const void* W, int ldw, int N, int K, void* out, hipStream_t s);
int launch_pack_w4(const void* W4, const unsigned char* S, int N, int K, void* W4P, unsigned char* SP, hipStream_t s);
int launch_gemv(int dtype, const GemvArgs& a, hipStream_t stream);
int launch_gemv_wait(int dtype, const GemvArgs& a, const unsigned* flags, unsigned epoch, int nflags, unsigned* err, int mode, hipStream_t s);
int launch_quant_fp8_rows(int dtype, const void* W, int ldw, int N, int K, void* W8, int ld8, float* scale, hipStream_t stream);
int launch_quant_mxfp4_rows(int dtype, const void* W, int ldw, int N, int K, void* W4, int ld4, unsigned char* S, hipStream_t stream);
void gemv_set_force_mfma(int v);
int gemv_get_force_mfma();
void gemm_set_autotune(int v);
int gemm_tune_load(const char* path);
int gemm_tune_dump(const char* path);
long gemm_tune_runs();
void model_set_ar_min_rows(int v);
void model_set_tp_f32(int v);
void model_set_pack_replica(int v);
void model_set_norm_in_gemv(int v);
void model_set_vit_fused(int v);
void model_set_tp_sp(int v);
int launch_fold_cols(int dtype, const void* W, const void* n, void* out, int rows, int cols, hipStream_t s);

int launch_layernorm(int dtype, const void* x, int ldx, const void* w, const void* b, void* y, int ldy, int rows, int H, float eps, hipStream_t stream);
int launch_rmsnorm(int dtype, const void* x, int ldx, const void* w, void* y, int ldy, int rows, int H, float eps, hipStream_t s, int pack_nb = 0);
int launch_rmsnorm_q8(int dtype, const void* x, int ldx, const void* w, void* y8, int ldy, float* scale, int rows, int H, float eps, hipStream_t s);
int launch_quant_rows_q8(int dtype, const void* x, int ldx, void* y8, int ldy, float* scale, int rows, int H, hipStream_t s);
int launch_resid_rmsnorm(int dtype, void* x, int ldx, const float* part, int ks, const void* w, void* xn, int ldn, int rows, int H, float eps,
                         hipStream_t s, int pack_nb = 0);
int launch_resid16_norm(int dtype, void* x, int ldx, const void* y, int ldy, const void* w, const void* b, void* xn, int ldn, int rows, int H, float eps,
                        hipStream_t s);
int launch_vit_qknorm(int dtype, void* qkv, int ld, const void* wq, const void* wk, int rows, int C, int C_total,
                      float eps, float q_scale, const float* sumsq_in, hipStream_t s, int only_k = 0);
int launch_vit_qk_sumsq(int dtype, const void* qkv, int ld, int rows, int C, float* sumsq_out, hipStream_t s);
int launch_vit_knorm_slots(int dtype, void* k, int ld, const void* wk, int rows, int C, int C_total, float eps, const float* stats, int stats_ld, int nslots,
                           float* sumsq_q, hipStream_t s);
struct AttnArgs {
  const void* Q; int64_t q_sb, q_sh, q_sr;
  const void* K; int64_t k_sb, k_sh, k_sr;
  const void* V; int64_t v_sb, v_sh, v_sr;
  void* O; int64_t o_sb, o_sh, o_sr;
  int batch, q_heads, kv_heads;
  int Sq, Skv;
  const int* kv_len;
  const int* kv_start;
  int causal;
  int q_pos0;
  float scale;
  int head_dim;
  const float* qn_sumsq = nullptr; int qn_stride = 0, qn_dim = 0; const void* qn_w = nullptr; float qn_eps = 0.f, qn_scale = 1.f;
};
int launch_attn_prefill(int dtype, const AttnArgs& a, hipStream_t s);
int launch_attn_uniform_rows(int dtype, const AttnArgs& a, hipStream_t s);
void attn_set_v2(int v);
void model_set_fuse_peer_norm(int v);
void attn_set_tpw(int v);
void attn_set_klds(int v);
void attn_set_dma(int v);
void attn_set_dma_slots(int v);
void attn_set_dma_rot(int v);
void attn_set_hsplit(int v);
void attn_set_mha_xcd(int v);
void attn_set_kg(int v);
void attn_set_peel(int v);
void attn_set_kv8_tpw(int v);
void attn_set_kv8_fuse(int v);
void model_set_extend_attn(int v);
bool attn_decode_kv8_fuses_rope(int batch, int kv_heads, int L, bool masked);
void attn_set_merge_mid_min(int v);
void attn_set_merge_dg(int v);
void gemv_set_norm_loop(int v);
void gemv_set_dyn(int v);
void gemv_set_skew(int v);
void gemv_set_rows_balance(int v);
void gemv_set_no_xs(int v);
void gemv_set_shard_shapes(int v);
void gemv_set_gu_rr(int v);
void gemv_set_longk_direct(int v);
void norm_set_wave(int v);
void model_set_ao_oproj(int v);
int gemv_get_shard_shapes();

struct AttnDecodeArgs {
  const void* Q; int64_t q_sb, q_sh;
  const void* K; int64_t k_sb, k_sh, k_sr;
  const void* V; int64_t v_sb, v_sh, v_sr;
  void* O; int64_t o_sb, o_sh;
  int batch, q_heads, kv_heads;
  int L;
  const int* kv_len;
  float scale;
  float* ws; size_t ws_bytes;
  const float* rope; int rope_max;
  const int* pos;
  const void* k_new; const void* v_new; int64_t new_sb;
  int o_pack_nb;
  const float* k_scale; const float* v_scale; int64_t scale_sb, scale_sh;
  void* k16_w = nullptr; void* v16_w = nullptr;
  const unsigned char* key_mask; int64_t mask_sb;
  unsigned* done_flags = nullptr; unsigned done_epoch = 0; int done_mode = 0;
// ... 213 lines not shown
```

### omchat_amd/csrc/model.hip

```cpp
#include "ctx.h"
#include <limits.h>
#include <math.h>
#include <string.h>
#include <algorithm>
#include <functional>
#include <string>
#include <unordered_map>
#include <vector>

static thread_local std::string g_err;
void omchat_set_error(const std::string& s) { g_err = s; }
extern "C" const char* omchat_last_error(void) { return g_err.c_str(); }
extern "C" const char* omchat_version(void) { return "omchat_hip 0.1 (gfx950)"; }

namespace {

__global__ void cast_from_f32_f16(const float* s, f16* d, int64_t n) {
  for (int64_t i = (int64_t)blockIdx.x * blockDim.x + threadIdx.x; i < n; i += (int64_t)gridDim.x * blockDim.x) d[i] = (f16)s[i];
}
__global__ void cast_from_f32_bf16(const float* s, bf16* d, int64_t n) {
  for (int64_t i = (int64_t)blockIdx.x * blockDim.x + threadIdx.x; i < n; i += (int64_t)gridDim.x * blockDim.x) d[i] = (bf16)s[i];
}
__global__ void add_positions_kernel(int* pos, int b, int d) {
  const int i = threadIdx.x;
// ... 322 lines not shown
  if (ctx->graph_ev_in) (void)hipEventDestroy(ctx->graph_ev_in);
  if (ctx->graph_ev_out) (void)hipEventDestroy(ctx->graph_ev_out);
  if (ctx->graph_stream) (void)hipStreamDestroy(ctx->graph_stream);
  for (hipEvent_t e : ctx->ev_chunk) if (e) (void)hipEventDestroy(e);
  for (hipEvent_t e : ctx->ev_ag) if (e) (void)hipEventDestroy(e);
  if (ctx->ev_comm_done) (void)hipEventDestroy(ctx->ev_comm_done);
  if (ctx->tp_f32_ws) (void)hipFree(ctx->tp_f32_ws);
  if (ctx->comm_stream) (void)hipStreamDestroy(ctx->comm_stream);
  if (ctx->stage_f32) hipFree(ctx->stage_f32);
  if (ctx->stage_t) hipFree(ctx->stage_t);
  ctx->beam.release(); ctx->group.release(); ctx->ext_ws.release(); ctx->pick.release();
  delete ctx;
}

extern "C" size_t omchat_device_bytes(omchat_ctx* ctx) { return ctx ? ctx->bytes : 0; }

extern "C" int omchat_load_tensor(omchat_ctx* ctx, const char* name, const void* data, const int64_t* shape, int ndim, int src_dtype) {
  OM_CHECK(ctx && name && data && shape, "null argument");
  auto it = ctx->routes.find(name);
  OM_CHECK(it != ctx->routes.end(), std::string("unknown tensor name: ") + name);
  Route& r = it->second;
  int64_t n = 1;
  for (int i = 0; i < ndim; ++i) n *= shape[i];
  OM_CHECK(n == r.rows * r.cols, std::string("shape mismatch for ") + name + ": expected " + std::to_string(r.rows * r.cols) +
                                     " elements, got " + std::to_string(n));
  {
    bool split_ok = r.rows == 1 || ndim == 1;
    int64_t lead = 1;
    for (int i = 0; i < ndim && !split_ok; ++i) { lead *= shape[i]; split_ok = lead == r.rows; }
    OM_CHECK(split_ok, std::string("shape mismatch for ") + name + ": expected [" + std::to_string(r.rows) + ", " + std::to_string(r.cols) + "]");
  }
  for (int f = 0; f < OMCHAT_WFMT_COUNT; ++f)
    if (f != OMCHAT_WFMT_16 && ctx->built(f)) ctx->wt[f].state = omchat_ctx::W_STALE;
  if (src_dtype == ctx->dt) return place(ctx, r, data);
  OM_CHECK(src_dtype == OMCHAT_F32, "source dtype must be the context dtype or OMCHAT_F32");
  TRY(ensure_stage(ctx, (size_t)n * 4, (size_t)n * 2));
  OM_HIP(hipMemcpy(ctx->stage_f32, data, (size_t)n * 4, hipMemcpyDefault));
  const int grid = (int)((n + 255) / 256 > 4096 ? 4096 : (n + 255) / 256);
  if (ctx->dt == OMCHAT_F16) hipLaunchKernelGGL(cast_from_f32_f16, dim3(grid), dim3(256), 0, 0, (const float*)ctx->stage_f32, (f16*)ctx->stage_t, n);
  else hipLaunchKernelGGL(cast_from_f32_bf16, dim3(grid), dim3(256), 0, 0, (const float*)ctx->stage_f32, (bf16*)ctx->stage_t, n);
  OM_LAUNCH_CHECK();
  OM_HIP(hipDeviceSynchronize());
  return place(ctx, r, ctx->stage_t);
}

static uint64_t fnv1a64(const std::string& s) {
  uint64_t h = 0xCBF29CE484222325ull;
  for (unsigned char ch : s) { h ^= ch; h *= 0x100000001B3ull; }
  return h;
}

extern "C" int omchat_fill_synthetic(omchat_ctx* ctx, uint64_t seed) {
  OM_CHECK(ctx, "null ctx");
  size_t maxn = 0;
  for (auto& kv : ctx->routes) maxn = std::max(maxn, (size_t)(kv.second.rows * kv.second.cols));
  TRY(ensure_stage(ctx, 16, maxn * 2));
  for (auto& kv : ctx->routes) {
    Route& r = kv.second;
    const int64_t n = r.rows * r.cols;
    const float scale = (float)((double)r.synth_std * sqrt(3.0));
    TRY(launch_fill_uniform(ctx->dt, ctx->stage_t, n, fnv1a64(kv.first) ^ seed, scale, r.synth_off, 0));
    OM_HIP(hipDeviceSynchronize());
    TRY(place(ctx, r, ctx->stage_t));
  }
  return 0;
}
// ... 463 lines not shown
  if (T.e.empty()) {
    std::vector<omchat_ctx::WRef> fresh(src.size());
    std::vector<void**> slots;
    std::vector<size_t> sizes;
    for (size_t j = 0; j < fresh.size(); ++j) {
      const size_t N = entry_shape(ctx, j).N, K = entry_shape(ctx, j).K;
      omchat_ctx::WRef& r = fresh[j];
      r.ldw = (int)(mx || mxp ? K / 2 : K);
      r.packed = p16 || mxp;
      slots.push_back(&r.W); sizes.push_back(p16 ? N * K * 2 : f8 ? N * K : N * (K / 2));
      if (f8) { slots.push_back((void**)&r.w_scale); sizes.push_back(N * 4); }
      if (mx || mxp) { slots.push_back((void**)&r.mx_scale); sizes.push_back(N * (K / 32)); }
    }
    if (ctx->alloc_group(slots, sizes)) {
      if (p16) { T.state = omchat_ctx::W_UNAVAILABLE; return 0; }
      if (mxp) omchat_set_error("omchat_enable_mxfp4_decode: the packed MXFP4 replica of mode 2 does not fit in device memory (hipMalloc failed)");
      return 2;
    }
    T.e.swap(fresh);
  }
  for (size_t j = 0; j < T.e.size(); ++j) {
    const int N = entry_shape(ctx, j).N, K = entry_shape(ctx, j).K;
    const omchat_ctx::WRef& w = src[j]; const omchat_ctx::WRef& r = T.e[j];
    if (f8) TRY(launch_quant_fp8_rows(ctx->dt, w.W, K, N, K, r.W, K, r.w_scale, nullptr));
    else if (mx) TRY(launch_quant_mxfp4_rows(ctx->dt, w.W, K, N, K, r.W, K / 2, r.mx_scale, nullptr));
    else if (mxp) TRY(launch_pack_w4(w.W, w.mx_scale, N, K, r.W, r.mx_scale, nullptr));
    else TRY(launch_pack_w(ctx->dt, w.W, K, N, K, r.W, nullptr));
  }
  OM_HIP(hipDeviceSynchronize());
  T.state = omchat_ctx::W_BUILT;
  return 0;
}

extern "C" int omchat_enable_fp8_decode(omchat_ctx* ctx, int on) {
  OM_CHECK(ctx, "null context");
  OM_CHECK(ctx->c.t_layers > 0, "context has no decoder");
  if (!on) { ctx->fp8_decode = false; return 0; }
  OM_CHECK(!ctx->mxfp4_mode, "MXFP4 decode is on: one weight format per step (omchat_enable_mxfp4_decode(ctx, 0) first)");
  TRY(build_replica(ctx, OMCHAT_WFMT_E4M3));
  ctx->fp8_decode = true;
  return 0;
}

extern "C" int omchat_enable_mxfp4_decode(omchat_ctx* ctx, int mode) {
  OM_CHECK(ctx, "null context");
  OM_CHECK(ctx->c.t_layers > 0, "context has no decoder");
  OM_CHECK(mode >= 0 && mode <= 2, "mode: 0 = off, 1 = batch-1 steps, 2 = steps of up to 32 rows as well");
  if (!mode) { ctx->mxfp4_mode = 0; return 0; }
  OM_CHECK(!ctx->fp8_decode, "fp8 decode is on: one weight format per step (omchat_enable_fp8_decode(ctx, 0) first)");
  OM_CHECK(ctx->tp_size == 1, "MXFP4 decode under tensor parallelism is not implemented");
  if (mode == 2) {
    const omchat_config& c = ctx->c;
    OM_CHECK(c.t_hidden % 64 == 0 && ctx->t_qdim % 64 == 0 && c.t_mlp % 64 == 0,
             "MXFP4 decode mode 2: the packed path needs hidden_size, heads x 128 and intermediate_size each a multiple of 64");
    OM_CHECK(ctx->t_qkvdim % 16 == 0 && c.t_hidden % 16 == 0 && c.t_vocab % 16 == 0,
             "MXFP4 decode mode 2: the packed path needs the qkv width, hidden_size and vocab_size each a multiple of 16");
  }
  TRY(build_replica(ctx, mode == 2 ? OMCHAT_WFMT_MXFP4_PACKED : OMCHAT_WFMT_MXFP4));
  ctx->mxfp4_mode = mode;
  return 0;
}

extern "C" int omchat_enable_fp8_kv(omchat_ctx* ctx, int on) {
  OM_CHECK(ctx, "null context");
  const omchat_config& c = ctx->c;
  OM_CHECK(c.t_layers > 0, "context has no decoder");
// ... 202 lines not shown

extern "C" int omchat_kv_read(omchat_ctx* ctx, int layer, int which, int pos0, int n, void* out, void* stream) {
  OM_CHECK(ctx && out, "null argument");
  const omchat_config& c = ctx->c;
  OM_CHECK(layer >= 0 && layer < c.t_layers && (which == 0 || which == 1) && pos0 >= 0 && n >= 1 && pos0 + n <= c.max_seq, "bad argument");
  const char* src = (const char*)(which ? ctx->vcache : ctx->kcache) + ((size_t)layer * ctx->cache_layer_stride() + (size_t)pos0 * 128) * 2;
  OM_HIP(hipMemcpy2DAsync(out, (size_t)n * 256, src, (size_t)ctx->cache_sh() * 2, (size_t)n * 256, (size_t)c.t_kv_heads, hipMemcpyDeviceToDevice,
                          (hipStream_t)stream));
  return 0;
}

extern "C" int omchat_decode_weight_format(int rows, int fp8_on, int mxfp4_mode, int packed16_ready, int geometry_ok, int* x_pack_nb) {
  const bool batched = rows >= 2 && rows <= 32;
  const int nb = batched && geometry_ok ? (rows > 16 ? 2 : 1) : 0;
  if (x_pack_nb) *x_pack_nb = nb;
  if (rows == 1) return fp8_on ? OMCHAT_WFMT_E4M3 : mxfp4_mode >= 1 ? OMCHAT_WFMT_MXFP4 : OMCHAT_WFMT_16;
  if (batched && mxfp4_mode == 2) return OMCHAT_WFMT_MXFP4_PACKED;
  return nb && packed16_ready ? OMCHAT_WFMT_16_PACKED : OMCHAT_WFMT_16;
}
static int step_format(const omchat_ctx* ctx, int rows, int* x_pack_nb = nullptr, bool assume_packed16 = false) {
  const omchat_config& c = ctx->c;
  return omchat_decode_weight_format(rows, ctx->fp8_decode, ctx->mxfp4_mode, assume_packed16 || ctx->built(OMCHAT_WFMT_16_PACKED),
                                     c.t_hidden % 64 == 0 && ctx->t_qdim % 64 == 0 && c.t_mlp % 64 == 0, x_pack_nb);
}
static bool is_mxfp4(int fmt) { return fmt == OMCHAT_WFMT_MXFP4 || fmt == OMCHAT_WFMT_MXFP4_PACKED; }

static int step_weights_ready(omchat_ctx* ctx, int rows) {
  const omchat_config& c = ctx->c;
  if (step_format(ctx, rows, nullptr, true) == OMCHAT_WFMT_16_PACKED && g_pack_replica && ctx->wt[OMCHAT_WFMT_16_PACKED].state != omchat_ctx::W_UNAVAILABLE &&
      !(ctx->t_qkvdim % 16 || c.t_hidden % 16 || c.t_vocab % 16))
    TRY(build_replica(ctx, OMCHAT_WFMT_16_PACKED));
  if (ctx->fp8_decode) TRY(build_replica(ctx, OMCHAT_WFMT_E4M3));
  if (ctx->mxfp4_mode) TRY(build_replica(ctx, ctx->mxfp4_mode == 2 ? OMCHAT_WFMT_MXFP4_PACKED : OMCHAT_WFMT_MXFP4));
  return 0;
}

static const char* const MX4_ROWS_MSG = "MXFP4 decode mode 2 streams steps of at most 32 rows (omchat_enable_mxfp4_decode(ctx, 0 or 1) first)";
static bool mx4_rows_ok(const omchat_ctx* ctx, int rows) { return ctx->mxfp4_mode != 2 || is_mxfp4(step_format(ctx, rows)); }

static int decode_body(omchat_ctx* ctx, const int32_t* tokens, int b, int Lmax, float* logits, int32_t* next_tokens, hipStream_t s, bool allow_prof,
                       bool exact_len = false, bool masked = false, int vL = -1, bool vsample = false) {
  const omchat_config& c = ctx->c;
  const int H = c.t_hidden, It = c.t_mlp, qkvd = ctx->t_qkvdim, qd = ctx->t_qdim;
  const bool lead = ctx->tp_rank == 0;
  void* x = ctx->tw_x;
  void* y = ctx->tw_x2;
  TRY(launch_gather_rows(ctx->dt, tokens, ctx->t_embed, nullptr, x, b, H, s));
  int pk = 0;
  const int fmt = step_format(ctx, b, &pk);
  OM_CHECK(fmt != OMCHAT_WFMT_MXFP4_PACKED || pk, "MXFP4 decode mode 2: geometry outside the packed path");
  const bool wq = fmt == OMCHAT_WFMT_E4M3 || is_mxfp4(fmt);
  const bool wpk = fmt == OMCHAT_WFMT_16_PACKED, mpk = fmt == OMCHAT_WFMT_MXFP4_PACKED;
  using WRef = omchat_ctx::WRef;
  enum { QKV = omchat_ctx::P_QKV, O = omchat_ctx::P_O, GU = omchat_ctx::P_GU, DOWN = omchat_ctx::P_DOWN };
  auto gemv_args = [&](const void* X, int ldx, const WRef& W, int K, void* Y, int ldy, int R, int N, const void* bias, const void* resid, int epi,
                       int ks, bool ypk) {
    GemvArgs g{X, ldx, nullptr, 0, Y, ldy, R, N, K, bias, resid, H, epi, 0, ks};
    use_weight(g, W);
    if (pk) { g.x_packed = 1; g.y_packed = ypk && epi == EPI_SWIGLU; }
    return g;
  };
  auto gemv = [&](const void* X, int ldx, const WRef& W, int K, void* Y, int ldy, int N, const void* bias, const void* resid, int epi,
                  bool ypk = false) -> int {
    for (int r0 = 0; r0 < b; r0 += 32) {
      const int R = std::min(32, b - r0);
      const GemvArgs g = gemv_args((const char*)X + (size_t)r0 * ldx * 2, ldx, W, K, (char*)Y + (size_t)r0 * ldy * 2, ldy, R, N, bias,
                                   resid ? (const char*)resid + (size_t)r0 * H * 2 : nullptr, epi, 0, ypk);
      TRY(launch_gemv(ctx->dt, g, s));
    }
    return 0;
  };
  auto gemv_partial = [&](const void* X, int ldx, const WRef& W, int K, int ks) -> int {
    OM_CHECK(b <= 32, "split-K decode path handles b <= 32");
    const GemvArgs g = gemv_args(X, ldx, W, K, ctx->tw_part, H, b, H, nullptr, nullptr, EPI_PARTIAL, ks, false);
    TRY(launch_gemv(ctx->dt, g, s));
    return 0;
  };
  const bool fused = b <= 32;
  auto ks_rows = [&](int K) { const int nch = cdiv(K, 512); return nch >= 16 ? std::min(DEC_KS_MAX, nch) : std::max(1, std::min(3, nch)); };
  auto ks_short = [&](int K) { return std::max(1, std::min(DEC_KS_MAX, (K / 64) / 16)); };
  const bool shard_ks = (gemv_get_shard_shapes() & 2) != 0;
  const int ks_o = b == 1 ? ks_rows(qd) : ((wpk || mpk) && qd == 3584 ? 2 : (shard_ks && qd / 64 <= 64) ? ks_short(qd) :
                                           std::max(1, std::min(DEC_KS_MAX, std::min(qd / 64, cdiv(512, cdiv(H, 16))))));
  const int ks_d = b == 1 ? ks_rows(It) : (shard_ks && It / 64 <= 64) ? ks_short(It) :
                                          std::max(1, std::min(DEC_KS_MAX, std::min(It / 64, 3 * cdiv(512, cdiv(H, 16)))));
  const bool tp1_like = ctx->tp_size == 1 || (OMCHAT_EXPERIMENTS && g_shard_as_tp1 && ctx->hook == omchat_allreduce_noop);
  const bool n2 = (g_norm_in_gemv & 1) && fused && b == 1 && tp1_like && qd <= 4096 && H <= 4096 && !gemv_get_force_mfma();
  const bool n1 = n2 && (g_norm_in_gemv & 2) && It <= 32768 && It % 8 == 0;
  const bool nb2 = OMCHAT_EXPERIMENTS && (g_norm_in_gemv & 4) && fused && wpk && ctx->tp_size == 1 && !wq && (qd >> 6) == 56 && (H >> 6) == 56 && qd % 64 == 0 &&
                   H / 16 <= device_cus() && (2 * It) / 32 >= 4 * device_cus();
  if (fused && !n1) TRY(launch_rmsnorm(ctx->dt, x, H, ctx->dl[0].ln1, ctx->tw_xn, H, b, H, c.t_eps, s, pk));
#if OMCHAT_EXPERIMENTS
  if ((g_ao_oproj & 16) && ctx->dbg_stamps) OM_HIP(hipMemsetAsync(ctx->dbg_stamps, 0, (size_t)c.t_layers * 256, s));
#endif
  for (int i = 0; i < c.t_layers; ++i) {
    auto& L = ctx->dl[i];
    const WRef* W = ctx->layer_w(fmt, i);
    const WRef* W16 = ctx->layer_w(OMCHAT_WFMT_16, i);
    char* kc = (char*)ctx->kcache + (size_t)i * ctx->cache_layer_stride() * 2;
    char* vc = (char*)ctx->vcache + (size_t)i * ctx->cache_layer_stride() * 2;
    if (!fused) TRY(launch_rmsnorm(ctx->dt, x, H, L.ln1, ctx->tw_xn, H, b, H, c.t_eps, s));
    if (g_decode_layer && n1 && exact_len && !masked && !wq && !(ctx->fp8_kv && ctx->kv8_valid) && ctx->dl_ws) {
      DecodeLayerArgs d{L.ln1, L.ln2, W16[QKV].W, L.bqkv, W16[O].W, W16[GU].W, W16[DOWN].W, kc, vc, ctx->cache_sh(), x, H, qd, ctx->t_kvdim, It, c.t_heads, c.t_kv_heads, Lmax,
                        ctx->rope, c.max_seq, c.t_eps, 0.08838834764831845f, ctx->dl_ws, ++ctx->fd_epoch, ctx->fd_err, 2000};
      if (decode_layer_ok(d)) {
        const bool mark_l = allow_prof && i == c.t_layers / 2;
        if (mark_l) ctx->prof_mark(OMCHAT_PROF_DECODE_GATEUP, s);
        TRY(launch_decode_layer(ctx->dt, d, s));
        if (mark_l) ctx->prof_mark(OMCHAT_PROF_DECODE_GATEUP, s);
        ++ctx->n_layer_launches;
        continue;
      }
      --ctx->fd_epoch;
    }
    if (n1) {
      GemvArgs g = gemv_args(x, H, W[QKV], H, ctx->tw_qkv, qkvd, 1, qkvd, L.bqkv, nullptr, EPI_NONE, 0, false);
      g.norm_w = L.ln1; g.norm_eps = c.t_eps;
      if (OMCHAT_EXPERIMENTS && (g_ao_oproj & 16) && ctx->dbg_stamps) g.dbg = ctx->dbg_stamps + (size_t)i * 32;
      TRY(launch_gemv(ctx->dt, g, s));
    } else {
      TRY(gemv(ctx->tw_xn, H, W[QKV], H, ctx->tw_qkv, qkvd, qkvd, L.bqkv, nullptr, EPI_NONE));
    }
    AttnDecodeArgs a{};
// ... 61 lines not shown
      TRY(launch_attn_decode(ctx->dt, a, s));
    }
    if (fuse_ao) {
    } else if (ao_oproj) {
      GemvArgs g = gemv_args(ctx->tw_ao, qd, W16[O], qd, x, H, 1, H, nullptr, x, EPI_RESID, 0, false);
      if ((g_ao_oproj & 16) && ctx->dbg_stamps) g.dbg = ctx->dbg_stamps + (size_t)i * 32;
      TRY(launch_gemv_wait(ctx->dt, g, (const unsigned*)ctx->fd_ws, ctx->fd_epoch, c.t_heads, ctx->fd_err, g_ao_oproj, s));
    } else if (n2 && OMCHAT_EXPERIMENTS && (g_ao_oproj & 16) && ctx->dbg_stamps && !wq) {
      GemvArgs g = gemv_args(ctx->tw_ao, qd, W16[O], qd, x, H, 1, H, nullptr, x, EPI_RESID, 0, false);
      g.dbg = ctx->dbg_stamps + (size_t)i * 32;
      TRY(launch_gemv(ctx->dt, g, s));
    } else if (n2) {
      TRY(gemv(ctx->tw_ao, qd, W[O], qd, x, H, H, nullptr, x, EPI_RESID));
    } else if (nb2) {
      GemvArgs g = gemv_args(ctx->tw_ao, qd, W[O], qd, x, H, b, H, nullptr, x, EPI_RESID, 0, false);
      g.y_pack = ctx->tw_xn;
      TRY(launch_gemv(ctx->dt, g, s));
    } else if (fused) {
      TRY(gemv_partial(ctx->tw_ao, qd, W[O], qd, ks_o));
      TRY(ctx->reduce_resid_rmsnorm(x, H, ctx->tw_part, ks_o, L.ln2, ctx->tw_xn, H, b, H, c.t_eps, pk, s));
    } else if (ctx->tp_size == 1) {
      TRY(gemv(ctx->tw_ao, qd, W[O], qd, x, H, H, nullptr, x, EPI_RESID));
    } else {
      TRY(gemv(ctx->tw_ao, qd, W[O], qd, y, H, H, nullptr, lead ? x : nullptr, lead ? EPI_RESID : EPI_NONE));
      TRY(ctx->allreduce(y, (size_t)b * H, s));
      std::swap(x, y);
    }
    if (!fused) TRY(launch_rmsnorm(ctx->dt, x, H, L.ln2, ctx->tw_xn, H, b, H, c.t_eps, s));
    const bool mark = allow_prof && i == c.t_layers / 2;
    if (mark) ctx->prof_mark(OMCHAT_PROF_DECODE_GATEUP, s);
    if (n2) {
      GemvArgs g = gemv_args(x, H, W[GU], H, ctx->tw_act, It, 1, 2 * It, nullptr, nullptr, EPI_SWIGLU, 0, false);
      g.norm_w = L.ln2; g.norm_eps = c.t_eps;
      if (ctx->dyn_ctr && !ctx->graph_on) g.dyn_ctr = ctx->dyn_ctr + (size_t)i * 65 * 64;
      if (OMCHAT_EXPERIMENTS && (g_ao_oproj & 16) && ctx->dbg_stamps) g.dbg = ctx->dbg_stamps + (size_t)i * 32;
      TRY(launch_gemv(ctx->dt, g, s));
    } else if (nb2) {
      GemvArgs g = gemv_args(ctx->tw_xn, H, W[GU], H, ctx->tw_act, It, b, 2 * It, nullptr, nullptr, EPI_SWIGLU, 0, true);
      g.norm_w = L.ln2; g.norm_eps = c.t_eps;
      TRY(launch_gemv(ctx->dt, g, s));
    } else {
      TRY(gemv(ctx->tw_xn, H, W[GU], H, ctx->tw_act, It, 2 * It, nullptr, nullptr, EPI_SWIGLU, true));
    }
    if (mark) ctx->prof_mark(OMCHAT_PROF_DECODE_GATEUP, s);
    if (n1 && OMCHAT_EXPERIMENTS && (g_ao_oproj & 16) && ctx->dbg_stamps && !wq) {
      GemvArgs g = gemv_args(ctx->tw_act, It, W16[DOWN], It, x, H, 1, H, nullptr, x, EPI_RESID, 0, false);
      g.dbg = ctx->dbg_stamps + (size_t)i * 32;
      TRY(launch_gemv(ctx->dt, g, s));
    } else if (n1) {
      TRY(gemv(ctx->tw_act, It, W[DOWN], It, x, H, H, nullptr, x, EPI_RESID));
    } else if (fused) {
      TRY(gemv_partial(ctx->tw_act, It, W[DOWN], It, ks_d));
      const void* nw = i + 1 < c.t_layers ? ctx->dl[i + 1].ln1 : ctx->t_norm;
      TRY(ctx->reduce_resid_rmsnorm(x, H, ctx->tw_part, ks_d, nw, ctx->tw_xn, H, b, H, c.t_eps, pk, s));
    } else if (ctx->tp_size == 1) {
      TRY(gemv(ctx->tw_act, It, W[DOWN], It, x, H, H, nullptr, x, EPI_RESID));
    } else {
      TRY(gemv(ctx->tw_act, It, W[DOWN], It, y, H, H, nullptr, lead ? x : nullptr, lead ? EPI_RESID : EPI_NONE));
      TRY(ctx->allreduce(y, (size_t)b * H, s));
      std::swap(x, y);
    }
  }
  if (!fused)   TRY(launch_rmsnorm(ctx->dt, x, H, ctx->t_norm, ctx->tw_xn, H, b, H, c.t_eps, s));
  float* lg = logits ? logits : ctx->tw_logits;
  if (n1) {
    GemvArgs g{x, H, nullptr, 0, lg, c.t_vocab, 1, c.t_vocab, H, nullptr, nullptr, 0, EPI_NONE, 1};
    use_weight(g, ctx->lm_w(fmt));
    g.norm_w = ctx->t_norm; g.norm_eps = c.t_eps;
    TRY(launch_gemv(ctx->dt, g, s));
  } else {
    TRY(lm_head_rows(ctx, ctx->tw_xn, b, lg, s, ctx->lm_w(fmt), fused && pk));
  }
  if (vL >= 0) TRY(pick_verify(ctx, lg, b, tokens, next_tokens, s, vsample));
  else if (next_tokens) TRY(pick_run(ctx, lg, b, next_tokens, s, true, tokens));
  else {
    hipLaunchKernelGGL(advance_lens_kernel, dim3(1), dim3(64 > b ? 64 : b), 0, s, ctx->d_pos, ctx->d_len, b);
    TRY(pick_feed(ctx, tokens, b, s));
  }
  OM_LAUNCH_CHECK();
  return 0;
}

static void destroy_graph(omchat_ctx::DecodeGraph& g) {
  if (g.exec) (void)hipGraphExecDestroy(g.exec);
  if (g.graph) (void)hipGraphDestroy(g.graph);
  g = omchat_ctx::DecodeGraph{};
}

void drop_decode_graphs(omchat_ctx* ctx) {
  for (auto& kv : ctx->graphs) destroy_graph(kv.second);
  ctx->graphs.clear();
}


extern "C" int omchat_enable_decode_graph(omchat_ctx* ctx, int on) {
  OM_CHECK(ctx, "null ctx");
  OM_CHECK(ctx->c.t_layers > 0, "context has no decoder");
  if (on && !ctx->graph_stream) {
    OM_HIP(hipStreamCreateWithFlags(&ctx->graph_stream, hipStreamNonBlocking));
    OM_HIP(hipEventCreateWithFlags(&ctx->graph_ev_in, hipEventDisableTiming));
    OM_HIP(hipEventCreateWithFlags(&ctx->graph_ev_out, hipEventDisableTiming));
    TRY(ctx->alloc((void**)&ctx->d_tok_in, (size_t)ctx->c.max_batch * 4));
    TRY(ctx->alloc((void**)&ctx->d_tok_out, (size_t)ctx->c.max_batch * 4));
  }
  ctx->graph_on = on != 0;
  return 0;
}

extern "C" int omchat_decode_graph_stats(omchat_ctx* ctx, long* steps, long* replays, long* captures) {
  OM_CHECK(ctx, "null ctx");
  if (steps) *steps = ctx->graph_steps;
  if (replays) *replays = ctx->graph_replays;
  if (captures) *captures = ctx->graph_captures;
  return 0;
}

extern "C" int omchat_decode_step(omchat_ctx* ctx, const int32_t* tokens, int b, float* logits, int32_t* next_tokens, void* stream) {
  OM_CHECK(ctx && tokens, "null argument");
  const omchat_config& c = ctx->c;
  OM_CHECK(c.t_layers > 0, "context has no decoder");
  OM_CHECK(b >= 1 && b <= c.max_batch, "batch exceeds max_batch");
  OM_CHECK(mx4_rows_ok(ctx, b), MX4_ROWS_MSG);
  int Lmax = 0;
  OM_CHECK(!ctx->left_padded, "per-sequence decode after a left-padded prefill: use omchat_decode_step_masked (the reference positions such a "
                              "batch with sum(mask) - 1 and a per-row key mask, omchat_arch.py:61-70; DESIGN.md section 7)");
  OM_CHECK(ctx->dec_mode != 2, "omchat_decode_step after omchat_decode_step_masked on the same prefill: the two place the cache rows differently");
  bool same_len = true;
  for (int i = 0; i < b; ++i) {
    OM_CHECK(ctx->h_len[i] >= 1, "decode before prefill");
    Lmax = std::max(Lmax, ctx->h_len[i] + 1);
    same_len = same_len && ctx->h_len[i] == ctx->h_len[0];
  }
  OM_CHECK(Lmax <= c.max_seq, "KV cache full (max_seq)");
  hipStream_t s = (hipStream_t)stream;
  GroupState& G = ctx->group;
  const bool grp = G.on();
  if (grp) {
    OM_CHECK(b == G.b * G.N && same_len, "a sampled group shares its prompt: a step takes all its b * N rows, of one length (omchat_group_begin with b = 0 first)");
    OM_CHECK(ctx->tp_size == 1 && !(ctx->fp8_kv && ctx->kv8_valid), "shared-prompt mode: one GPU, 16-bit KV cache");
    Lmax = std::min(c.max_seq, G.P + (Lmax - G.P + 255) / 256 * 256);
    const size_t need = attn_shared_ws_bytes(G.b, G.N, c.t_heads, c.t_kv_heads, G.P, Lmax);
    if (need > G.ws.cap) TRY(ctx->grow(G.ws, attn_shared_ws_bytes(G.b, G.N, c.t_heads, c.t_kv_heads, G.P, std::min(c.max_seq, Lmax + 768))));
  }
  TRY(step_weights_ready(ctx, b));
  TRY(pick_admit(ctx, next_tokens != nullptr, true));
  ctx->graph_steps++;
  const bool graph = ctx->graph_on && ctx->tp_size == 1 && b <= 32 && !(ctx->prof_on && ctx->graph_steps % 8 == 0);
  if (!graph) {
    TRY(decode_body(ctx, tokens, b, Lmax, logits, next_tokens, s, true, same_len && !grp));
  } else {
    const int fmt = step_format(ctx, b);
    omchat_ctx::DecodeGraph& g = ctx->graphs[b * 8 + (is_mxfp4(fmt) ? 4 : 0) + (fmt == OMCHAT_WFMT_E4M3 ? 2 : 0) + ((ctx->fp8_kv && ctx->kv8_valid) ? 1 : 0) +
                                             (grp ? (1 << 20) : 0)];
    hipStream_t gs = ctx->graph_stream;
    OM_HIP(hipEventRecord(ctx->graph_ev_in, s));
    OM_HIP(hipStreamWaitEvent(gs, ctx->graph_ev_in, 0));
    OM_HIP(hipMemcpyAsync(ctx->d_tok_in, tokens, (size_t)b * 4, hipMemcpyDeviceToDevice, gs));
    if (!g.exec || Lmax > g.cap_len || (grp && (Lmax != g.cap_len || G.N != g.grp_N || G.P != g.grp_P || G.ws.p != g.grp_ws))) {
      destroy_graph(g);
      const int cap = grp ? Lmax : std::min(c.max_seq, (Lmax + 1024 + 63) / 64 * 64);
      OM_HIP(hipStreamBeginCapture(gs, hipStreamCaptureModeThreadLocal));
      const int rc = decode_body(ctx, ctx->d_tok_in, b, cap, ctx->tw_logits, ctx->d_tok_out, gs, false);
      hipGraph_t graph_h = nullptr;
      const hipError_t e = hipStreamEndCapture(gs, &graph_h);
      if (rc) { if (graph_h) (void)hipGraphDestroy(graph_h); return rc; }
      OM_HIP(e);
      g.graph = graph_h;
      OM_HIP(hipGraphInstantiate(&g.exec, g.graph, nullptr, nullptr, 0));
      g.cap_len = cap;
      if (grp) { g.grp_N = G.N; g.grp_P = G.P; g.grp_ws = G.ws.p; }
      ctx->graph_captures++;
    }
    OM_HIP(hipGraphLaunch(g.exec, gs));
    ctx->graph_replays++;
    if (next_tokens) OM_HIP(hipMemcpyAsync(next_tokens, ctx->d_tok_out, (size_t)b * 4, hipMemcpyDeviceToDevice, gs));
    if (logits) OM_HIP(hipMemcpyAsync(logits, ctx->tw_logits, (size_t)b * c.t_vocab * 4, hipMemcpyDeviceToDevice, gs));
    OM_HIP(hipEventRecord(ctx->graph_ev_out, gs));
    OM_HIP(hipStreamWaitEvent(s, ctx->graph_ev_out, 0));
  }
  for (int i = 0; i < b; ++i) ctx->h_len[i] += 1;
  ctx->dec_mode = 1;
  return 0;
}

extern "C" int omchat_decode_verify(omchat_ctx* ctx, const int32_t* tokens, int T, float* logits, int32_t* picks, int* n_accept, int flags,
                                    void* stream) {
// ... 270 lines not shown
```

### omchat_amd/engine.py

```python
import ctypes as C
import numpy as np

from . import _lib
from ._lib import OmchatConfig, check, ptr, cur_stream
from .config import OmChatConfig


def _torch():
    import torch
    return torch


GROUP_SHARE_P_MIN = 2048


def group_share_refusal(fp8_kv, tp_size, q_heads, kv_heads, N):
    if fp8_kv:
        return "the e4m3 KV cache"
    if tp_size != 1:
        return "tensor parallelism"
    if not 2 <= N <= 16 or N * (q_heads // max(1, kv_heads)) > 128:
        return "N outside 2 <= N <= 16 and N * (q heads per kv head) <= 128"
    return None

# ... 123 lines not shown
        rs, ag = C.c_long(0), C.c_long(0)
        check(self.lib.omchat_ctx_sp_stats(self.h, C.byref(rs), C.byref(ag)))
        return dict(peer_allreduces=a.value, rccl_allreduces=b.value, sp_reduce_scatters=rs.value, sp_all_gathers=ag.value)

    def enable_fp8_decode(self, on=True):
        check(self.lib.omchat_enable_fp8_decode(self.h, int(on)))

    def enable_mxfp4_decode(self, on=True, batched=False):
        check(self.lib.omchat_enable_mxfp4_decode(self.h, (2 if batched else 1) if on else 0))
        self._mxfp4_decode = bool(on)
        self._mxfp4_batched = bool(on) and bool(batched)

    def enable_fp8_kv(self, on=True):
        check(self.lib.omchat_enable_fp8_kv(self.h, int(on)))
        self._fp8_kv = bool(on)
        self._prefix = None

    def masked_decode_supported(self):
        return self.tp_size == 1

    def enable_fp8_prefill(self, on=True):
        check(self.lib.omchat_enable_fp8_prefill(self.h, int(on)))
        self._fp8_prefill = bool(on)
        self._prefix = None

    def enable_decode_graph(self, on=True):
        check(self.lib.omchat_enable_decode_graph(self.h, int(on)))

    def decode_graph_stats(self):
        st, rp, cp = C.c_long(0), C.c_long(0), C.c_long(0)
        check(self.lib.omchat_decode_graph_stats(self.h, C.byref(st), C.byref(rp), C.byref(cp)))
        return dict(steps=st.value, replays=rp.value, captures=cp.value)

    def prof_enable(self, on=True):
        check(self.lib.omchat_prof_enable(self.h, int(on)))

    def prof_read(self, cat, reset=True):
        ms, n = C.c_double(0), C.c_long(0)
        check(self.lib.omchat_prof_read(self.h, cat, C.byref(ms), C.byref(n), int(reset)))
        return ms.value, n.value

    def device_bytes(self):
        return int(self.lib.omchat_device_bytes(self.h))

    def _px(self, pixels):
        torch = _torch()
        if pixels.dim() != 4 or pixels.shape[1] != 3:
            raise ValueError(f"wrong pixel_values size: {tuple(pixels.shape)}")
        s = self.cfg.vision["image_size"]
        if pixels.shape[2] != s or pixels.shape[3] != s:
            raise ValueError(f"expected {s}x{s} tiles, got {tuple(pixels.shape[2:])}")
        return pixels.to(device=self.device, dtype=self.torch_dtype).contiguous()

    def vit_forward(self, pixels, select_layer=-1, select_feature="patch"):
        torch = _torch()
        if select_feature not in ("patch", "cls_patch"):
            raise ValueError(f"Unexpected select feature: {select_feature}")
        px = self._px(pixels)
        n = px.shape[0]
        keep = select_feature == "cls_patch"
        out = torch.empty(n, self.ntok + (1 if keep else 0), self.cfg.vision["hidden_size"], dtype=self.torch_dtype, device=self.device)
        check(self.lib.omchat_vit_forward(self.h, ptr(px), n, select_layer, int(keep), ptr(out), cur_stream()))
        return out

    def projector_forward(self, x):
        torch = _torch()
# ... 356 lines not shown
```

Before: 343.6.

## Add lossless 12-bit compressed bf16 weight format for single-row decode GEMVs

Adds an encoder that packs bf16 weights into 12 bits per value. It stores the low byte plus a 3-bit exponent offset from a per-row top exponent and the sign, and keeps up to 32 per-row patch entries for values that do not fit. New GEMV paths (rows_norm and longk) decode these in registers with byte perms. They are used by default for gate/up and LM head (roles mask 5) in batch-1 bf16 decode. The aim is to cut weight memory traffic in memory-bound decode by about a quarter, at the cost of extra decode ALU work, patch handling, and a second copy of the weights in device memory. Rows that overflow the patch budget fall back to plain bf16.

```diff
diff --git a/include/omchat_hip.h b/include/omchat_hip.h
--- a/include/omchat_hip.h
+++ b/include/omchat_hip.h
@@ -115,6 +115,7 @@
 
 int omchat_enable_decode_graph(omchat_ctx* ctx, int on);
 int omchat_decode_graph_stats(omchat_ctx* ctx, long* steps, long* replays, long* captures);
+int omchat_bf16x12_stats(omchat_ctx* ctx, int* roles, long* launches, int* coded);
 
 int omchat_enable_fp8_decode(omchat_ctx* ctx, int on);
 
@@ -187,6 +188,9 @@
                               const void* bias, int epi, int out_f32, int ksplit, void* stream);
 int omchat_op_gemv_mxfp4_packed(int dtype, const void* X, int ldx, const void* W4, const void* S, void* Y, int ldy, int b, int N, int K,
                                 const void* bias, int epi, int out_f32, int ksplit, int y_packed, void* stream);
+int omchat_op_encode_bf16x12(const void* W, int N, int K, void* coded, void* top, void* cnt, void* patch, void* over, void* stream);
+int omchat_op_gemv_bf16x12(const void* X, const void* coded, const void* top, const void* cnt, const void* patch, void* Y, int N, int K,
+                           const void* norm_w, float eps, const void* resid, int epi, int out_f32, void* stream);
 int omchat_op_pack_w(int dtype, const void* W, int ldw, int N, int K, void* out, void* stream);
 int omchat_op_pack_w4(const void* W4, const void* S, int N, int K, void* W4P, void* SP, void* stream);
 int omchat_op_gemv_prepacked(int dtype, const void* XP, const void* WP, const void* SP, void* Y, int ldy, int b, int N, int K, const void* bias,
diff --git a/omchat_amd/_lib.py b/omchat_amd/_lib.py
--- a/omchat_amd/_lib.py
+++ b/omchat_amd/_lib.py
@@ -99,6 +99,7 @@
     "omchat_enable_fp8_kv": (_i, [_vp, _i]),
     "omchat_enable_fp8_prefill": (_i, [_vp, _i]),
     "omchat_enable_decode_graph": (_i, [_vp, _i]),
+    "omchat_bf16x12_stats": (_i, [_vp, C.POINTER(_i), C.POINTER(C.c_long), C.POINTER(_i)]),
     "omchat_decode_graph_stats": (_i, [_vp, C.POINTER(C.c_long), C.POINTER(C.c_long), C.POINTER(C.c_long)]),
     "omchat_op_quant_fp8": (_i, [_i, _vp, _i, _i, _vp, _vp, _vp]),
     "omchat_op_gemv_fp8": (_i, [_i, _vp, _vp, _vp, _vp, _i, _i, _vp, _vp, _i, _i, _i, _vp]),
@@ -111,6 +112,8 @@
     "omchat_op_pack_w": (_i, [_i, _vp, _i, _i, _i, _vp, _vp]),
     "omchat_op_pack_w4": (_i, [_vp, _vp, _i, _i, _vp, _vp, _vp]),
     "omchat_op_gemv_prepacked": (_i, [_i, _vp, _vp, _vp, _vp, _i, _i, _i, _i, _vp, _i, _i, _i, _i, _vp]),
+    "omchat_op_encode_bf16x12": (_i, [_vp, _i, _i, _vp, _vp, _vp, _vp, _vp, _vp]),
+    "omchat_op_gemv_bf16x12": (_i, [_vp, _vp, _vp, _vp, _vp, _vp, _i, _i, _vp, _f, _vp, _i, _i, _vp]),
     "omchat_op_gemv_mxfp4_norm": (_i, [_i, _vp, _vp, _vp, _vp, _i, _i, _vp, _f, _vp, _i, _i, _vp]),
     "omchat_op_rmsnorm": (_i, [_i, _vp, _vp, _vp, _i, _i, _f, _vp]),
     "omchat_op_resid_rmsnorm": (_i, [_i, _vp, _i, _vp, _i, _vp, _vp, _i, _i, _i, _f, _i, _vp]),
diff --git a/omchat_amd/csrc/capi.hip b/omchat_amd/csrc/capi.hip
--- a/omchat_amd/csrc/capi.hip
+++ b/omchat_amd/csrc/capi.hip
@@ -95,6 +95,7 @@
   if (key == 47) { attn_set_kv8_tpw(value); return 0; }
   if (key == 48) { attn_set_kv8_fuse(value); return 0; }
   if (key == 49) { model_set_extend_attn(value); return 0; }
+  if (key == 50) { model_set_x12_roles(value); return 0; }
   if (key == 38) { gemv_set_gu_rr(value); return 0; }
   if (key == 39) { gemv_set_longk_direct(value); return 0; }
   if (key == 40) { norm_set_wave(value); return 0; }
@@ -796,6 +797,18 @@
   return launch_gemv(dtype, g, S(stream));
 }
 
+extern "C" int omchat_op_encode_bf16x12(const void* W, int N, int K, void* coded, void* top, void* cnt, void* patch, void* over, void* stream) {
+  return launch_encode_bf16x12(W, K, N, K, coded, (unsigned char*)top, (unsigned char*)cnt, (unsigned*)patch, (int*)over, S(stream));
+}
+extern "C" int omchat_op_gemv_bf16x12(const void* X, const void* coded, const void* top, const void* cnt, const void* patch, void* Y, int N, int K,
+                                      const void* norm_w, float eps, const void* resid, int epi, int out_f32, void* stream) {
+  OM_CHECK(X && coded && top && cnt && patch && Y, "null argument");
+  GemvArgs g{X, K, coded, K / 2 * 3, Y, N, 1, N, K, nullptr, resid, N, epi, out_f32};
+  g.norm_w = norm_w; g.norm_eps = eps;
+  g.x12_top = (const unsigned char*)top; g.x12_cnt = (const unsigned char*)cnt; g.x12_patch = (const unsigned*)patch;
+  return launch_gemv(OMCHAT_BF16, g, S(stream));
+}
+
 extern "C" int omchat_op_attn_prefill_d(int dtype, const void* q, const void* k, const void* v, void* out, int b, int Sq, int Skv, int Hq,
                                         int Hkv, int D, const int32_t* kv_len, int causal, int q_pos0, float scale, void* stream) {
   AttnArgs a{};
diff --git a/omchat_amd/csrc/ctx.h b/omchat_amd/csrc/ctx.h
--- a/omchat_amd/csrc/ctx.h
+++ b/omchat_amd/csrc/ctx.h
@@ -120,6 +120,12 @@
   const WRef* layer_w(int fmt, int layer) const { return &wt[fmt].e[(size_t)layer * 4]; }
   const WRef& lm_w(int fmt) const { return wt[fmt].e.back(); }
   bool built(int fmt) const { return wt[fmt].state == W_BUILT; }
+  enum X12Role { X12_GU = 0, X12_DOWN = 1, X12_LM = 2, X12_ROLES = 3 };
+  struct X12Ref { void* W = nullptr; unsigned char* top = nullptr; unsigned char* cnt = nullptr; unsigned* patch = nullptr; bool ok = false; };
+  struct X12Table { std::vector<X12Ref> e; int state = W_ABSENT; };
+  X12Table x12[X12_ROLES];
+  int* x12_over = nullptr;
+  long x12_launches[X12_ROLES] = {0, 0, 0};
   bool fp8_decode = false;
   int mxfp4_mode = 0;
   void *k8cache = nullptr, *v8cache = nullptr;
@@ -309,6 +315,11 @@
   g.W = w.W; g.ldw = w.ldw; g.w_scale = w.w_scale; g.mx_scale = w.mx_scale; g.w_packed = w.packed;
 }
 
+inline void use_weight_x12(GemvArgs& g, const omchat_ctx::X12Ref& r, int K) {
+  g.W = r.W; g.ldw = K / 2 * 3; g.w_scale = nullptr; g.mx_scale = nullptr; g.w_packed = 0;
+  g.x12_top = r.top; g.x12_cnt = r.cnt; g.x12_patch = r.patch;
+}
+
 void drop_decode_graphs(omchat_ctx* ctx);
 
 int pick_alloc(omchat_ctx* ctx, int rows);
diff --git a/omchat_amd/csrc/gemv.hip b/omchat_amd/csrc/gemv.hip
--- a/omchat_amd/csrc/gemv.hip
+++ b/omchat_amd/csrc/gemv.hip
@@ -14,11 +14,14 @@
   void* y_pack;
   unsigned long long* dbg;
   const unsigned char* mx_s;
+  const unsigned char* x12_top;
+  const unsigned char* x12_cnt;
+  const unsigned* x12_patch;
 #if OMCHAT_EXPERIMENTS
   int xskew;
 #endif
 };
-constexpr int WF_16 = 0, WF_E4M3 = 1, WF_MX4 = 2;
+constexpr int WF_16 = 0, WF_E4M3 = 1, WF_MX4 = 2, WF_X12 = 3;
 #if OMCHAT_EXPERIMENTS
 #define OM_DBG_MIN(slot, cond) do { if (p.dbg && (cond) && threadIdx.x == 0) atomicMax(p.dbg + (slot), ~wall_clock64()); } while (0)
 #define OM_DBG_MAX(slot, cond) do { if (p.dbg && (cond) && threadIdx.x == 0) atomicMax(p.dbg + (slot), wall_clock64()); } while (0)
@@ -654,8 +657,81 @@
 template <int WF> struct RwW { typedef rw_u32x4 type; };
 template <> struct RwW<WF_E4M3> { typedef rw_u32x2 type; };
 template <> struct RwW<WF_MX4> { typedef rw_u32x2 type; };
+struct X12W { rw_u32x2 lo; unsigned nib; };
+template <> struct RwW<WF_X12> { typedef X12W type; };
+struct X12Row {
+  unsigned top_raw, cnt_raw;
+  unsigned pv;
+  unsigned tlo, thi;
+  int cnt, pi;
+};
+__device__ __forceinline__ X12W x12_ldw(const GemvP& p, size_t row, int chunk, int lane) {
+  const unsigned char* rec = (const unsigned char*)p.W + row * (size_t)p.ldw + (size_t)chunk * 768;
+  const unsigned lo_off = 8u * (unsigned)lane, nib_off = 512u + 4u * (unsigned)lane;
+  X12W w;
+  w.lo = __builtin_nontemporal_load(reinterpret_cast<const rw_u32x2*>(rec + lo_off));
+  w.nib = __builtin_nontemporal_load(reinterpret_cast<const unsigned*>(rec + nib_off));
+  return w;
+}
+__device__ __forceinline__ void x12_row_load(X12Row& s, const GemvP& p, size_t row, int lane) {
+  s.top_raw = p.x12_top[row];
+  s.cnt_raw = p.x12_cnt[row];
+  s.pv = p.x12_patch[row * 32 + (lane & 31)];
+}
+__device__ __forceinline__ void x12_row_finish(X12Row& s) {
+  const int t = __builtin_amdgcn_readfirstlane((int)s.top_raw) - 7;
+  s.cnt = __builtin_amdgcn_readfirstlane((int)s.cnt_raw);
+  s.pi = 0;
+  s.tlo = ((unsigned)((t + 1) & 0x7f) << 8) | ((unsigned)((t + 2) & 0x7f) << 16) | ((unsigned)((t + 3) & 0x7f) << 24);
+  s.thi = (unsigned)((t + 4) & 0x7f) | ((unsigned)((t + 5) & 0x7f) << 8) | ((unsigned)((t + 6) & 0x7f) << 16) | ((unsigned)((t + 7) & 0x7f) << 24);
+}
+__device__ __forceinline__ rw_u32x4 x12_decode(const X12W& w, const X12Row& s) {
+  const unsigned n = w.nib;
+  const unsigned c0 = n & 0x07070707u, c1 = (n >> 4) & 0x07070707u;
+  unsigned h0 = __builtin_amdgcn_perm(s.thi, s.tlo, c0), h1 = __builtin_amdgcn_perm(s.thi, s.tlo, c1);
+  h0 |= (n & 0x08080808u) << 4;
+  h1 |= n & 0x80808080u;
+  rw_u32x4 r;
+  r.x = __builtin_amdgcn_perm(h0, w.lo.x, 0x05010400u);
+  r.y = __builtin_amdgcn_perm(h0, w.lo.x, 0x07030602u);
+  r.z = __builtin_amdgcn_perm(h1, w.lo.y, 0x05010400u);
+  r.w = __builtin_amdgcn_perm(h1, w.lo.y, 0x07030602u);
+  return r;
+}
+__device__ __forceinline__ void x12_apply(rw_u32x4& w, unsigned e, int lane) {
+  const unsigned k = e >> 16, i = k & 7u, sh = (i & 1u) * 16u;
+  const unsigned keep = ~(0xffffu << sh), ins = (e & 0xffffu) << sh;
+  const bool mine = lane == (int)((k >> 3) & 63u);
+  w.x = (mine && (i >> 1) == 0u) ? ((w.x & keep) | ins) : w.x;
+  w.y = (mine && (i >> 1) == 1u) ? ((w.y & keep) | ins) : w.y;
+  w.z = (mine && (i >> 1) == 2u) ? ((w.z & keep) | ins) : w.z;
+  w.w = (mine && (i >> 1) == 3u) ? ((w.w & keep) | ins) : w.w;
+}
+template <int G>
+__device__ __forceinline__ void x12_group(rw_u32x4 (&wd)[G], const X12W* w, X12Row& s, int chunk0, int nch, int lane) {
+#pragma unroll
+  for (int i = 0; i < G; ++i) wd[i] = x12_decode(w[i], s);
+  while (s.pi < s.cnt) {
+    const unsigned e = (unsigned)__builtin_amdgcn_readlane((int)s.pv, s.pi);
+    const int ch = (int)(e >> 25) - chunk0;
+    if (ch >= G) break;
+#pragma unroll
+    for (int i = 0; i < G; ++i) if (ch == i) x12_apply(wd[i], e, lane);
+    ++s.pi;
+  }
+  if (chunk0 + G > nch) {
+    for (int j = 0; j < s.cnt; ++j) {
+      const unsigned e = (unsigned)__builtin_amdgcn_readlane((int)s.pv, j);
+      if ((e >> 19) != 0u) break;
+#pragma unroll
+      for (int i = 0; i < G; ++i) if (chunk0 + i >= nch) x12_apply(wd[i], e, 0);
+    }
+  }
+}
+
 template <typename T, int WF>
 __device__ __forceinline__ typename RwW<WF>::type rw_ldw(const GemvP& p, size_t row, int k) {
+  if constexpr (WF == WF_X12) return x12_ldw(p, row, k >> 9, (k >> 3) & 63); else
   if constexpr (WF == WF_E4M3) {
     return __builtin_nontemporal_load(reinterpret_cast<const rw_u32x2*>((const unsigned char*)p.W + row * p.ldw + k));
   } else if constexpr (WF == WF_MX4) {
@@ -889,7 +965,8 @@
     for (int c = 0; c < NCH; ++c) {
       int k = c * 512 + lane * 8;
       k = k < p.K ? k : 0;
-      w[r][c] = rw_ldw<T, F8>(p, (size_t)rows[r], k);
+      if constexpr (F8 == WF_X12) w[r][c] = x12_ldw(p, (size_t)rows[r], c, lane);
+      else w[r][c] = rw_ldw<T, F8>(p, (size_t)rows[r], k);
     }
   float e_bias[RR], e_scale[R];
   {
@@ -910,6 +987,11 @@
 #pragma unroll
       for (int r = 0; r < R; ++r) e_scale[r] = p.w_scale[rows[r]];
     }
+  }
+  X12Row xst[F8 == WF_X12 ? R : 1];
+  if constexpr (F8 == WF_X12) {
+#pragma unroll
+    for (int r = 0; r < R; ++r) x12_row_load(xst[r], p, (size_t)rows[r], lane);
   }
   __builtin_amdgcn_sched_barrier(0);
   float ss = 0.f;
@@ -949,9 +1031,25 @@
 #pragma unroll
   for (int r = 0; r < R; ++r) {
     float a = 0.f;
+    if constexpr (F8 == WF_X12) x12_row_finish(xst[r]);
 #pragma unroll
     for (int c = 0; c < NCH; ++c) {
-      a = rw_dotw<T, F8>(w[r][c], xr[c], a);
+      if constexpr (F8 != WF_X12) a = rw_dotw<T, F8>(w[r][c], xr[c], a);
+    }
+    if constexpr (F8 == WF_X12) {
+      constexpr int G0 = NCH < 4 ? NCH : 4, G1 = NCH - G0;
+      {
+        rw_u32x4 wd[G0];
+        x12_group<G0>(wd, &w[r][0], xst[r], 0, NCH, lane);
+#pragma unroll
+        for (int c = 0; c < G0; ++c) a = rw_dot8<T>(wd[c], xr[c], a);
+      }
+      if constexpr (G1 > 0) {
+        rw_u32x4 wd[G1];
+        x12_group<G1>(wd, &w[r][G0], xst[r], G0, NCH, lane);
+#pragma unroll
+        for (int c = 0; c < G1; ++c) a = rw_dot8<T>(wd[c], xr[G0 + c], a);
+      }
     }
 #pragma unroll
     for (int o = 32; o > 0; o >>= 1) a += __shfl_xor(a, o, 64);
@@ -981,6 +1079,8 @@
 __global__ __launch_bounds__(WAVES * 64) void gemv_rows_norm_kernel(GemvP p) { gemv_rows_norm_body<T, EPI, RR, NCH, F8 ? WF_E4M3 : WF_16, WAVES>(p); }
 template <typename T, int EPI, int RR, int NCH, int WAVES = 4>
 __global__ __launch_bounds__(WAVES * 64) void gemv_rows_norm_mx4_kernel(GemvP p) { gemv_rows_norm_body<T, EPI, RR, NCH, WF_MX4, WAVES>(p); }
+template <typename T, int EPI, int RR, int NCH>
+__global__ __launch_bounds__(256) void gemv_rows_norm_x12_kernel(GemvP p) { gemv_rows_norm_body<T, EPI, RR, NCH, WF_X12, 4>(p); }
 
 template <typename T, int EPI, int NCH, int F8>
 __device__ __forceinline__ void gemv_rows_norm_loop_body(const GemvP& p, int per_wg, unsigned skew) {
@@ -1280,19 +1380,36 @@
     for (int c = 0; c < 8; ++c) {
       int k = (pass * 8 + c) * 512 + lane * 8;
       k = k < p.K ? k : 0;
-      w[c] = rw_ldw<T, F8>(p, (size_t)row, k);
+      if constexpr (F8 == WF_X12) w[c] = x12_ldw(p, (size_t)row, pass * 8 + c < nch ? pass * 8 + c : 0, pass * 8 + c < nch ? lane : 0);
+      else w[c] = rw_ldw<T, F8>(p, (size_t)row, k);
     }
   };
   float acc = 0.f;
+  X12Row xst;
   auto dots = [&](wreg_t (&w)[8], int pass) {
-#pragma unroll
-    for (int c = 0; c < 8; ++c) {
-      const rw_u32x4 xr = *reinterpret_cast<const rw_u32x4*>(xs + (pass * 8 + c) * 512 + lane * 8);
-      acc = rw_dotw<T, F8>(w[c], xr, acc);
+    if constexpr (F8 == WF_X12) {
+      constexpr int G = 2;
+#pragma unroll
+      for (int h = 0; h < 8 / G; ++h) {
+        rw_u32x4 wd[G];
+        x12_group<G>(wd, &w[G * h], xst, pass * 8 + G * h, nch, lane);
+#pragma unroll
+        for (int c = 0; c < G; ++c) {
+          const rw_u32x4 xr = *reinterpret_cast<const rw_u32x4*>(xs + (pass * 8 + G * h + c) * 512 + lane * 8);
+          acc = rw_dot8<T>(wd[c], xr, acc);
+        }
+      }
+    } else {
+#pragma unroll
+      for (int c = 0; c < 8; ++c) {
+        const rw_u32x4 xr = *reinterpret_cast<const rw_u32x4*>(xs + (pass * 8 + c) * 512 + lane * 8);
+        acc = rw_dotw<T, F8>(w[c], xr, acc);
+      }
     }
   };
   wreg_t wa[8], wb[8], wc[8];
   load_w(wa, 0);
+  if constexpr (F8 == WF_X12) x12_row_load(xst, p, (size_t)row, lane);
   if (npass > 1) load_w(wb, 1);
   if (npass > 2) load_w(wc, 2);
   const float e_bias_raw = tof(((const T*)(p.bias ? p.bias : p.X))[p.bias ? row : 0]);
@@ -1306,6 +1423,7 @@
     *reinterpret_cast<rw_u32x4*>(xs + i * 8) = v;
   }
   __syncthreads();
+  if constexpr (F8 == WF_X12) x12_row_finish(xst);
   for (int ps = 0; ps < npass; ps += 3) {
     if (ps > 0 && ps + 2 < npass) load_w(wc, ps + 2);
     dots(wa, ps);
@@ -1333,6 +1451,8 @@
 __global__ __launch_bounds__(512) void gemv_rows_longk_kernel(GemvP p, int rows_per_wg) { gemv_rows_longk_body<T, F8 ? WF_E4M3 : WF_16>(p, rows_per_wg); }
 template <typename T>
 __global__ __launch_bounds__(512) void gemv_rows_longk_mx4_kernel(GemvP p, int rows_per_wg) { gemv_rows_longk_body<T, WF_MX4>(p, rows_per_wg); }
+template <typename T>
+__global__ __launch_bounds__(512) void gemv_rows_longk_x12_kernel(GemvP p, int rows_per_wg) { gemv_rows_longk_body<T, WF_X12>(p, rows_per_wg); }
 
 #if OMCHAT_EXPERIMENTS
 template <typename T, int F8>
@@ -1419,7 +1539,14 @@
   const int grid = cdiv(p.N, rpw);
   const int npass = (cdiv(p.K, 512) + 7) / 8;
   const size_t lds = (size_t)npass * 8 * 512 * 2;
-  if (p.mx_s) {
+  if (p.x12_top) {
+    if constexpr (std::is_same<T, bf16>::value) {
+      static PerDeviceOnce set;
+      auto k = gemv_rows_longk_x12_kernel<T>;
+      if (set.first()) OM_HIP(hipFuncSetAttribute((const void*)k, hipFuncAttributeMaxDynamicSharedMemorySize, 64 * 1024));
+      hipLaunchKernelGGL(k, dim3(grid), dim3(64 * rpw), lds, s, p, rpw);
+    }
+  } else if (p.mx_s) {
     static PerDeviceOnce set;
     auto k = gemv_rows_longk_mx4_kernel<T>;
     if (set.first()) OM_HIP(hipFuncSetAttribute((const void*)k, hipFuncAttributeMaxDynamicSharedMemorySize, 64 * 1024));
@@ -1502,6 +1629,26 @@
   }
 }
 
+template <int EPI, int NCH>
+void launch_rows_norm_x12_n(const GemvP& p, hipStream_t s) {
+  constexpr int RR = EPI == EPI_SWIGLU ? 1 : 4;
+  const int n_out = EPI == EPI_SWIGLU ? p.N / 2 : p.N;
+  hipLaunchKernelGGL((gemv_rows_norm_x12_kernel<bf16, EPI, RR, NCH>), dim3(cdiv(cdiv(n_out, RR), 4)), dim3(256), 0, s, p);
+}
+template <int EPI>
+void launch_rows_norm_x12(const GemvP& p, hipStream_t s) {
+  switch (p.K / 512) {
+    case 1: launch_rows_norm_x12_n<EPI, 1>(p, s); break;
+    case 2: launch_rows_norm_x12_n<EPI, 2>(p, s); break;
+    case 3: launch_rows_norm_x12_n<EPI, 3>(p, s); break;
+    case 4: launch_rows_norm_x12_n<EPI, 4>(p, s); break;
+    case 5: launch_rows_norm_x12_n<EPI, 5>(p, s); break;
+    case 6: launch_rows_norm_x12_n<EPI, 6>(p, s); break;
+    case 7: launch_rows_norm_x12_n<EPI, 7>(p, s); break;
+    default: launch_rows_norm_x12_n<EPI, 8>(p, s); break;
+  }
+}
+
 template <typename T, int EPI, int RR, int F8>
 void launch_rows_r(const GemvP& p, hipStream_t s) {
   const int n_out = EPI == EPI_SWIGLU ? p.N / 2 : p.N;
@@ -1556,7 +1703,7 @@
 int launch_t(const GemvArgs& a, hipStream_t s) {
   const int ks = a.ksplit > 1 ? a.ksplit : 1;
   GemvP p{a.X, a.W, a.Y, a.bias, a.resid, a.ldx, a.ldw, a.ldy, a.ldr, a.b, a.N, a.K, a.out_f32, ks, a.w_scale, a.y_packed, a.norm_w, a.norm_eps,
-          (unsigned*)a.dyn_ctr, a.y_pack, a.dbg, a.mx_scale};
+          (unsigned*)a.dyn_ctr, a.y_pack, a.dbg, a.mx_scale, a.x12_top, a.x12_cnt, a.x12_patch};
   if (a.norm_w && a.x_packed && !(a.w_packed && ks == 1 && (a.K >> 6) == 56 && a.epi == EPI_SWIGLU && a.N % 32 == 0 && !g_gemv_no_xs)) {
     omchat_set_error("launch_gemv: the in-register RMSNorm on packed x exists for the x-stationary gate|up form only (packed W, K = 3584, no split-K)");
     return 1;
@@ -1654,6 +1801,21 @@
     OM_LAUNCH_CHECK();
     return 0;
   }
+  if (a.x12_top) {
+    const bool ok = std::is_same<T, bf16>::value && a.b == 1 && !a.x_packed && !a.w_packed && ks == 1 && a.K >= 512 && a.K % 512 == 0 &&
+                    a.ldw == a.K / 2 * 3 && a.x12_cnt && a.x12_patch && !a.w_scale && !a.mx_scale && !a.force_mfma && !g_gemv_force_mfma;
+    const bool norm = ok && a.norm_w && (a.epi == EPI_SWIGLU || a.epi == EPI_NONE) && a.K <= RW_MAXC * 512;
+    const bool longk = ok && !a.norm_w && a.epi == EPI_RESID && !a.out_f32 && a.K > RW_MAXC * 512 && a.K <= 32768;
+    if (!norm && !longk) {
+      omchat_set_error("launch_gemv: bf16x12 weights: bf16, b == 1, K % 512 == 0, and norm_w with EPI_SWIGLU / EPI_NONE (K <= 4096) or EPI_RESID on 4096 < K <= 32768");
+      return 1;
+    }
+    if (longk) { const int rc = launch_rows_longk<T>(p, s); if (rc) return rc; }
+    else if (a.epi == EPI_SWIGLU) launch_rows_norm_x12<EPI_SWIGLU>(p, s);
+    else launch_rows_norm_x12<EPI_NONE>(p, s);
+    OM_LAUNCH_CHECK();
+    return 0;
+  }
   if (a.b == 1 && !a.x_packed && a.epi == EPI_RESID && ks == 1 && !a.out_f32 && a.K > RW_MAXC * 512 && a.K % 8 == 0 && a.K <= 32768 &&
       ((!a.force_mfma && !g_gemv_force_mfma) || a.mx_scale)) {
     const int rc = launch_rows_longk<T>(p, s);
@@ -1717,6 +1879,9 @@
 void gemv_set_longk_direct(int v) { g_gemv_longk_direct = v; }
 void gemv_set_skew(int v) { g_gemv_skew = (unsigned)v; }
 void gemv_set_rows_balance(int v) { g_gemv_rows_balance = v; }
+int gemv_x12_default_forms() {
+  return ((g_gemv_norm_loop & 1) == 0 && g_gemv_gu_rr == 1 && g_gemv_skew == 0u ? 1 : 0) | (g_gemv_longk_direct == 0 ? 2 : 0) | ((g_gemv_norm_loop & 8) == 0 ? 4 : 0);
+}
 
 namespace {
 template <typename T>
@@ -1801,6 +1966,81 @@
   if (dtype == OMCHAT_F16) hipLaunchKernelGGL(quant_mxfp4_rows_kernel<f16>, dim3(cdiv(N, 4)), dim3(256), 0, s, (const f16*)W, ldw, N, K, (unsigned char*)W4, ld4, S);
   else if (dtype == OMCHAT_BF16) hipLaunchKernelGGL(quant_mxfp4_rows_kernel<bf16>, dim3(cdiv(N, 4)), dim3(256), 0, s, (const bf16*)W, ldw, N, K, (unsigned char*)W4, ld4, S);
   else { omchat_set_error("launch_quant_mxfp4_rows: bad dtype"); return 1; }
+  OM_LAUNCH_CHECK();
+  return 0;
+}
+
+namespace {
+__global__ __launch_bounds__(64) void encode_bf16x12_kernel(const unsigned short* __restrict__ W, int ldw, int N, int K, unsigned char* __restrict__ coded,
+                                                            unsigned char* __restrict__ top, unsigned char* __restrict__ cnt, unsigned* __restrict__ patch,
+                                                            int* __restrict__ over) {
+  const int lane = threadIdx.x, n = blockIdx.x;
+  const unsigned short* w = W + (size_t)n * ldw;
+  int t = 0;
+  for (int k = lane * 8; k < K; k += 512) {
+    const rw_u32x4 v = *reinterpret_cast<const rw_u32x4*>(w + k);
+    const unsigned u[4] = {v.x, v.y, v.z, v.w};
+#pragma unroll
+    for (int i = 0; i < 8; ++i) {
+      const int e = (int)((u[i >> 1] >> (16 * (i & 1) + 7)) & 0xffu);
+      if (e != 0xff) t = max(t, e >> 1);
+    }
+  }
+#pragma unroll
+  for (int o = 32; o > 0; o >>= 1) t = max(t, __shfl_xor(t, o, 64));
+  unsigned char* row = coded + (size_t)n * (size_t)(K / 512) * 768;
+  int total = 0;
+  for (int c = 0; c < K / 512; ++c) {
+    const int k0 = c * 512 + lane * 8;
+    const rw_u32x4 v = *reinterpret_cast<const rw_u32x4*>(w + k0);
+    const unsigned u[4] = {v.x, v.y, v.z, v.w};
+    unsigned lo0 = 0, lo1 = 0, nib = 0, mm = 0;
+#pragma unroll
+    for (int i = 0; i < 8; ++i) {
+      const unsigned h = (u[i >> 1] >> (16 * (i & 1))) & 0xffffu;
+      const int e = (int)((h >> 7) & 0xffu), e71 = e >> 1, cc = e71 - (t - 7);
+      const bool hit = e != 0xff && (e71 == 0 || cc >= 1);
+      const unsigned code = e71 == 0 ? 0u : (unsigned)cc;
+      if (hit) {
+        if (i < 4) lo0 |= (h & 0xffu) << (8 * i); else lo1 |= (h & 0xffu) << (8 * (i - 4));
+        nib |= (((h >> 15) << 3) | code) << (8 * (i & 3) + 4 * (i >> 2));
+      } else {
+        mm |= 1u << i;
+      }
+    }
+    const rw_u32x2 lo = {lo0, lo1};
+    *reinterpret_cast<rw_u32x2*>(row + (size_t)c * 768 + lane * 8) = lo;
+    *reinterpret_cast<unsigned*>(row + (size_t)c * 768 + 512 + lane * 4) = nib;
+    if (__ballot(mm != 0u)) {
+      const int pc = __popc(mm);
+      int inc = pc;
+#pragma unroll
+      for (int o = 1; o < 64; o <<= 1) { const int y = __shfl_up(inc, o, 64); if (lane >= o) inc += y; }
+      int off = total + inc - pc;
+#pragma unroll
+      for (int i = 0; i < 8; ++i) {
+        if ((mm >> i) & 1u) {
+          const unsigned h = (u[i >> 1] >> (16 * (i & 1))) & 0xffffu;
+          if (off < 32) patch[(size_t)n * 32 + off] = ((unsigned)(k0 + i) << 16) | h;
+          ++off;
+        }
+      }
+      total += __shfl(inc, 63, 64);
+    }
+  }
+  if (lane < 32 && lane >= total) patch[(size_t)n * 32 + lane] = 0u;
+  if (lane == 0) {
+    top[n] = (unsigned char)t;
+    cnt[n] = (unsigned char)(total > 32 ? 33 : total);
+    if (total > 32) *over = 1;
+  }
+}
+}
+
+int launch_encode_bf16x12(const void* W, int ldw, int N, int K, void* coded, unsigned char* top, unsigned char* cnt, unsigned* patch, int* over, hipStream_t s) {
+  OM_CHECK(W && coded && top && cnt && patch && over, "null argument");
+  OM_CHECK(N >= 1 && K >= 512 && K % 512 == 0 && K < 65536 && ldw % 8 == 0 && ldw >= K, "bf16x12: K a multiple of 512 below 65536, ldw % 8 == 0");
+  hipLaunchKernelGGL(encode_bf16x12_kernel, dim3(N), dim3(64), 0, s, (const unsigned short*)W, ldw, N, K, (unsigned char*)coded, top, cnt, patch, over);
   OM_LAUNCH_CHECK();
   return 0;
 }
diff --git a/omchat_amd/csrc/kernels.h b/omchat_amd/csrc/kernels.h
--- a/omchat_amd/csrc/kernels.h
+++ b/omchat_amd/csrc/kernels.h
@@ -76,7 +76,12 @@
   void* y_pack = nullptr;
   unsigned long long* dbg = nullptr;
   const unsigned char* mx_scale = nullptr;
-};
+  const unsigned char* x12_top = nullptr;
+  const unsigned char* x12_cnt = nullptr;
+  const unsigned* x12_patch = nullptr;
+};
+int launch_encode_bf16x12(const void* W, int ldw, int N, int K, void* coded, unsigned char* top, unsigned char* cnt, unsigned* patch, int* over,
+                          hipStream_t stream);
 int launch_pack_x(int dtype, const void* X, int ldx, int b, int K, void* out, hipStream_t s);
 int launch_pack_w(int dtype, const void* W, int ldw, int N, int K, void* out, hipStream_t s);
 int launch_pack_w4(const void* W4, const unsigned char* S, int N, int K, void* W4P, unsigned char* SP, hipStream_t s);
@@ -142,6 +147,8 @@
 void attn_set_kv8_tpw(int v);
 void attn_set_kv8_fuse(int v);
 void model_set_extend_attn(int v);
+void model_set_x12_roles(int v);
+int gemv_x12_default_forms();
 bool attn_decode_kv8_fuses_rope(int batch, int kv_heads, int L, bool masked);
 void attn_set_merge_mid_min(int v);
 void attn_set_merge_dg(int v);
diff --git a/omchat_amd/csrc/model.hip b/omchat_amd/csrc/model.hip
--- a/omchat_amd/csrc/model.hip
+++ b/omchat_amd/csrc/model.hip
@@ -378,6 +378,7 @@
   }
   for (int f = 0; f < OMCHAT_WFMT_COUNT; ++f)
     if (f != OMCHAT_WFMT_16 && ctx->built(f)) ctx->wt[f].state = omchat_ctx::W_STALE;
+  for (auto& t : ctx->x12) if (t.state == omchat_ctx::W_BUILT) t.state = omchat_ctx::W_STALE;
   if (src_dtype == ctx->dt) return place(ctx, r, data);
   OM_CHECK(src_dtype == OMCHAT_F32, "source dtype must be the context dtype or OMCHAT_F32");
   TRY(ensure_stage(ctx, (size_t)n * 4, (size_t)n * 2));
@@ -907,6 +908,56 @@
   return 0;
 }
 
+int g_x12_roles = 5;
+void model_set_x12_roles(int v) { g_x12_roles = v & 7; }
+
+static int x12_step_mask(const omchat_ctx* ctx, int rows, int fmt) {
+  if (rows != 1 || fmt != OMCHAT_WFMT_16 || ctx->dt != OMCHAT_BF16 || ctx->tp_size != 1) return 0;
+  return g_x12_roles & gemv_x12_default_forms();
+}
+
+static int build_x12(omchat_ctx* ctx, int role) {
+  omchat_ctx::X12Table& T = ctx->x12[role];
+  if (T.state == omchat_ctx::W_BUILT || T.state == omchat_ctx::W_UNAVAILABLE) return 0;
+  const omchat_config& c = ctx->c;
+  const int H = c.t_hidden, It = c.t_mlp, L = c.t_layers;
+  const bool lm = role == omchat_ctx::X12_LM, down = role == omchat_ctx::X12_DOWN;
+  const size_t N = lm ? c.t_vocab : down ? H : 2 * (size_t)It, K = down ? It : H, n = lm ? 1 : L;
+  const bool k_ok = K % 512 == 0 && (down ? (K > 4096 && K <= 32768) : K <= 4096);
+  if (!k_ok || omchat_weights_missing(ctx) != 0) { if (!k_ok) T.state = omchat_ctx::W_UNAVAILABLE; return 0; }
+  if (T.e.empty()) {
+    std::vector<omchat_ctx::X12Ref> fresh(n);
+    std::vector<void**> slots;
+    std::vector<size_t> sizes;
+    for (auto& r : fresh) {
+      slots.push_back(&r.W); sizes.push_back(N * (K / 2 * 3));
+      slots.push_back((void**)&r.top); sizes.push_back(N);
+      slots.push_back((void**)&r.cnt); sizes.push_back(N);
+      slots.push_back((void**)&r.patch); sizes.push_back(N * 32 * 4);
+    }
+    int* over = nullptr;
+    if (!ctx->x12_over) { slots.push_back((void**)&over); sizes.push_back((size_t)std::max(L, 1) * 4); }
+    if (ctx->alloc_group(slots, sizes)) { T.state = omchat_ctx::W_UNAVAILABLE; return 0; }
+    if (over) ctx->x12_over = over;
+    T.e.swap(fresh);
+  }
+  OM_HIP(hipDeviceSynchronize());
+  OM_HIP(hipMemset(ctx->x12_over, 0, n * 4));
+  for (size_t j = 0; j < n; ++j) {
+    const void* W = lm ? ctx->lm_w(OMCHAT_WFMT_16).W : ctx->layer_w(OMCHAT_WFMT_16, (int)j)[down ? omchat_ctx::P_DOWN : omchat_ctx::P_GU].W;
+    const omchat_ctx::X12Ref& r = T.e[j];
+    TRY(launch_encode_bf16x12(W, (int)K, (int)N, (int)K, r.W, r.top, r.cnt, r.patch, ctx->x12_over + j, nullptr));
+  }
+  OM_HIP(hipDeviceSynchronize());
+  std::vector<int> over(n);
+  OM_HIP(hipMemcpy(over.data(), ctx->x12_over, n * 4, hipMemcpyDeviceToHost));
+  bool moved = false;
+  for (size_t j = 0; j < n; ++j) { moved = moved || (T.state == omchat_ctx::W_STALE && T.e[j].ok != !over[j]); T.e[j].ok = !over[j]; }
+  if (moved) drop_decode_graphs(ctx);
+  T.state = omchat_ctx::W_BUILT;
+  return 0;
+}
+
 extern "C" int omchat_enable_fp8_decode(omchat_ctx* ctx, int on) {
   OM_CHECK(ctx, "null context");
   OM_CHECK(ctx->c.t_layers > 0, "context has no decoder");
@@ -1175,6 +1226,8 @@
     TRY(build_replica(ctx, OMCHAT_WFMT_16_PACKED));
   if (ctx->fp8_decode) TRY(build_replica(ctx, OMCHAT_WFMT_E4M3));
   if (ctx->mxfp4_mode) TRY(build_replica(ctx, ctx->mxfp4_mode == 2 ? OMCHAT_WFMT_MXFP4_PACKED : OMCHAT_WFMT_MXFP4));
+  const int x12m = x12_step_mask(ctx, rows, step_format(ctx, rows));
+  for (int role = 0; role < omchat_ctx::X12_ROLES; ++role) if (x12m >> role & 1) TRY(build_x12(ctx, role));
   return 0;
 }
 
@@ -1232,6 +1285,11 @@
   const bool n1 = n2 && (g_norm_in_gemv & 2) && It <= 32768 && It % 8 == 0;
   const bool nb2 = OMCHAT_EXPERIMENTS && (g_norm_in_gemv & 4) && fused && wpk && ctx->tp_size == 1 && !wq && (qd >> 6) == 56 && (H >> 6) == 56 && qd % 64 == 0 &&
                    H / 16 <= device_cus() && (2 * It) / 32 >= 4 * device_cus();
+  const int x12m = n1 ? x12_step_mask(ctx, b, fmt) : 0;
+  auto x12_of = [&](int role, size_t j) -> const omchat_ctx::X12Ref* {
+    const omchat_ctx::X12Table& T = ctx->x12[role];
+    return ((x12m >> role) & 1) && T.state == omchat_ctx::W_BUILT && T.e[j].ok ? &T.e[j] : nullptr;
+  };
   if (fused && !n1) TRY(launch_rmsnorm(ctx->dt, x, H, ctx->dl[0].ln1, ctx->tw_xn, H, b, H, c.t_eps, s, pk));
 #if OMCHAT_EXPERIMENTS
   if ((g_ao_oproj & 16) && ctx->dbg_stamps) OM_HIP(hipMemsetAsync(ctx->dbg_stamps, 0, (size_t)c.t_layers * 256, s));
@@ -1359,6 +1417,7 @@
     if (n2) {
       GemvArgs g = gemv_args(x, H, W[GU], H, ctx->tw_act, It, 1, 2 * It, nullptr, nullptr, EPI_SWIGLU, 0, false);
       g.norm_w = L.ln2; g.norm_eps = c.t_eps;
+      if (const auto* r = x12_of(omchat_ctx::X12_GU, i)) { use_weight_x12(g, *r, H); ++ctx->x12_launches[omchat_ctx::X12_GU]; }
       if (ctx->dyn_ctr && !ctx->graph_on) g.dyn_ctr = ctx->dyn_ctr + (size_t)i * 65 * 64;
       if (OMCHAT_EXPERIMENTS && (g_ao_oproj & 16) && ctx->dbg_stamps) g.dbg = ctx->dbg_stamps + (size_t)i * 32;
       TRY(launch_gemv(ctx->dt, g, s));
@@ -1373,6 +1432,11 @@
     if (n1 && OMCHAT_EXPERIMENTS && (g_ao_oproj & 16) && ctx->dbg_stamps && !wq) {
       GemvArgs g = gemv_args(ctx->tw_act, It, W16[DOWN], It, x, H, 1, H, nullptr, x, EPI_RESID, 0, false);
       g.dbg = ctx->dbg_stamps + (size_t)i * 32;
+      TRY(launch_gemv(ctx->dt, g, s));
+    } else if (n1 && x12_of(omchat_ctx::X12_DOWN, i)) {
+      GemvArgs g = gemv_args(ctx->tw_act, It, W[DOWN], It, x, H, 1, H, nullptr, x, EPI_RESID, 0, false);
+      use_weight_x12(g, *x12_of(omchat_ctx::X12_DOWN, i), It);
+      ++ctx->x12_launches[omchat_ctx::X12_DOWN];
       TRY(launch_gemv(ctx->dt, g, s));
     } else if (n1) {
       TRY(gemv(ctx->tw_act, It, W[DOWN], It, x, H, H, nullptr, x, EPI_RESID));
@@ -1393,6 +1457,7 @@
   if (n1) {
     GemvArgs g{x, H, nullptr, 0, lg, c.t_vocab, 1, c.t_vocab, H, nullptr, nullptr, 0, EPI_NONE, 1};
     use_weight(g, ctx->lm_w(fmt));
+    if (const auto* r = x12_of(omchat_ctx::X12_LM, 0)) { use_weight_x12(g, *r, H); ++ctx->x12_launches[omchat_ctx::X12_LM]; }
     g.norm_w = ctx->t_norm; g.norm_eps = c.t_eps;
     TRY(launch_gemv(ctx->dt, g, s));
   } else {
@@ -1431,6 +1496,18 @@
     TRY(ctx->alloc((void**)&ctx->d_tok_out, (size_t)ctx->c.max_batch * 4));
   }
   ctx->graph_on = on != 0;
+  return 0;
+}
+
+extern "C" int omchat_bf16x12_stats(omchat_ctx* ctx, int* roles, long* launches, int* coded) {
+  OM_CHECK(ctx, "null context");
+  if (roles) *roles = g_x12_roles;
+  for (int r = 0; r < omchat_ctx::X12_ROLES; ++r) {
+    if (launches) launches[r] = ctx->x12_launches[r];
+    int n = 0;
+    if (ctx->x12[r].state == omchat_ctx::W_BUILT) for (const auto& e : ctx->x12[r].e) n += e.ok ? 1 : 0;
+    if (coded) coded[r] = n;
+  }
   return 0;
 }
 
@@ -1478,7 +1555,7 @@
   } else {
     const int fmt = step_format(ctx, b);
     omchat_ctx::DecodeGraph& g = ctx->graphs[b * 8 + (is_mxfp4(fmt) ? 4 : 0) + (fmt == OMCHAT_WFMT_E4M3 ? 2 : 0) + ((ctx->fp8_kv && ctx->kv8_valid) ? 1 : 0) +
-                                             (grp ? (1 << 20) : 0)];
+                                             (grp ? (1 << 20) : 0) + (x12_step_mask(ctx, b, fmt) << 21)];
     hipStream_t gs = ctx->graph_stream;
     OM_HIP(hipEventRecord(ctx->graph_ev_in, s));
     OM_HIP(hipStreamWaitEvent(gs, ctx->graph_ev_in, 0));
diff --git a/omchat_amd/engine.py b/omchat_amd/engine.py
--- a/omchat_amd/engine.py
+++ b/omchat_amd/engine.py
@@ -179,6 +179,11 @@
         check(self.lib.omchat_decode_graph_stats(self.h, C.byref(st), C.byref(rp), C.byref(cp)))
         return dict(steps=st.value, replays=rp.value, captures=cp.value)
 
+    def bf16x12_stats(self):
+        roles, launches, coded = C.c_int(0), (C.c_long * 3)(), (C.c_int * 3)()
+        check(self.lib.omchat_bf16x12_stats(self.h, C.byref(roles), launches, coded))
+        return dict(roles=roles.value, launches=list(launches), coded=list(coded))
+
     def prof_enable(self, on=True):
         check(self.lib.omchat_prof_enable(self.h, int(on)))
 
```

After: 377.9 (median of 6 runs). +10.0%, better.
